# qiutang98/chord

Measured on AMD Instinct MI355X. Metric: Gtri/s into 4K 64-bit visbuffer, higher is better.
Workload: dtype f32+u64; 1 GPU; street_4k_hzb; scene_triangles_lod0=2799616, objects=352, hzb=True, cull=flat, parallelism=single

## Files before the change

chord_amd/csrc/chordvis_abi.cpp:

```cpp

#include "device_layer.h"
#include "material_tables.h"

#include <algorithm>
#include <cmath>
#include <cstddef>
#include <cstdio>
#include <cstring>

using namespace chord;

namespace chord {

int fail(ChordCtx* ctx, int code, const char* what, hipError_t e)
{
    if (ctx) {
        char buf[512];
        if (e != hipSuccess) std::snprintf(buf, sizeof(buf), "%s: %s (%d)", what, hipGetErrorString(e), (int)e);
        else std::snprintf(buf, sizeof(buf), "%s", what);
        ctx->lastError = buf;
    }
    return code;
}

}

namespace {

template <typename T>
int dalloc(ChordCtx* c, T** p, size_t count)
{
    if (*p) { (void)hipFree(*p); *p = nullptr; }
    if (count == 0) count = 1;
    CHORD_HIP(c, hipMalloc((void**)p, count * sizeof(T)));
    return CHORDVIS_OK;
}

template <typename T>
void dfree(T*& p) { if (p) { (void)hipFree((void*)p); p = nullptr; } }

uint32_t tex_block_bytes(uint32_t format)
{
    if (format == CHORD_TEXFMT_BC1_RGB || format == CHORD_TEXFMT_BC4) return 8u;
    if (format == CHORD_TEXFMT_BC3 || format == CHORD_TEXFMT_BC5) return 16u;
    return 0u;
}
#define CHORD_TEXFMT_NAMES "0 (RGBA8), 1 (BC1_RGB), 2 (BC3), 3 (BC4), 4 (BC5)"

struct TexDecodeJob {
    struct Copy { const uint8_t* host; uint64_t offset, bytes; };
    std::vector<chord::DTexLevelRec> recs;
    std::vector<Copy> copies;
    uint64_t stagingBytes = 0;
    uint32_t blocks = 0;

    void add(const ChordTexture& tx, uint32_t dst)
    {
        const uint32_t bb = tex_block_bytes(tx.format);
        const uint64_t offset = (stagingBytes + 15ull) & ~15ull;
        uint64_t bytes = 0;
        for (uint32_t l = 0; l < tx.mipCount; l++) {
            const uint32_t w = std::max(1u, tx.width >> l), h = std::max(1u, tx.height >> l), bw = (w + 3u) / 4u, bh = (h + 3u) / 4u;
            recs.push_back(chord::DTexLevelRec{blocks, (uint32_t)((offset + bytes) / 8u), dst, w, h, bw, tx.format, 0u});
            blocks += bw * bh; bytes += (uint64_t)bw * bh * bb; dst += w * h;
        }
        copies.push_back(Copy{tx.rgba8, offset, bytes});
        stagingBytes = offset + bytes;
    }

    int run(ChordCtx* c, const char* who, uint32_t* texels, uint8_t* alpha, bool alphaOnly)
    {
        if (recs.empty()) return CHORDVIS_OK;
        if (stagingBytes / 8u > 0xFFFFFFFFull) return fail(c, CHORDVIS_E_CAPACITY, "texture decode: more than 32 GiB of compressed texture levels in one upload");
        const uint32_t count = (uint32_t)recs.size();
        recs.push_back(chord::DTexLevelRec{blocks, 0u, 0u, 0u, 0u, 1u, 0u, 0u});
        uint8_t* dStaging = nullptr;
        chord::DTexLevelRec* dRecs = nullptr;
        hipError_t e = hipMalloc((void**)&dStaging, stagingBytes);
        if (e == hipSuccess) e = hipMalloc((void**)&dRecs, recs.size() * sizeof(recs[0]));
        if (e == hipSuccess) e = hipMemcpy(dRecs, recs.data(), recs.size() * sizeof(recs[0]), hipMemcpyHostToDevice);
        for (size_t i = 0; i < copies.size() && e == hipSuccess; i++)
            e = hipMemcpy(dStaging + copies[i].offset, copies[i].host, copies[i].bytes, hipMemcpyHostToDevice);
        if (e == hipSuccess) {
            chord::launch_texture_decode(c, dRecs, count, blocks, dStaging, texels, alpha, alphaOnly);
            e = hipGetLastError();
            const hipError_t es = hipStreamSynchronize(c->stream);
            if (e == hipSuccess) e = es;
        }
        if (dStaging) (void)hipFree(dStaging);
        if (dRecs) (void)hipFree(dRecs);
        return e == hipSuccess ? CHORDVIS_OK : fail(c, CHORDVIS_E_HIP, who, e);
    }
};

void record(ChordCtx* c, int tag) { chord::stamp(c, tag); }

void begin_frame_stamps(ChordCtx* c)
{
    c->frameLaunchBase = c->launchCount;
    c->stampThisFrame = c->timers && (c->frameIndex % c->timerPeriod) == 0;
    c->frameIndex++;
    if (!c->stampThisFrame) return;
    if (c->timers == 1) { c->stampTags.clear(); c->framesStamped = 0; }
    c->framesStamped++;
    chord::stamp(c, S_FRAME_BEGIN);
}

int alloc_hzb(ChordCtx* c, HzbBuffers& h)
{
    ChordHZBDesc d;
    if (chordvis_hzb_desc(c->width, c->height, &d) != CHORDVIS_OK) return fail(c, CHORDVIS_E_INVALID, "render size unsupported for HZB");
    h.desc = d;
    h.valid = false; h.uploaded = false;
    int rc;
    if ((rc = dalloc(c, &h.minTexels, d.totalTexels))) return rc;
    if ((rc = dalloc(c, &h.maxTexels, d.totalTexels))) return rc;
    if ((rc = dalloc(c, &h.validRange, 2))) return rc;
    CHORD_HIP(c, hipMemsetAsync(h.minTexels, 0, sizeof(uint16_t) * d.totalTexels, c->stream));
    CHORD_HIP(c, hipMemsetAsync(h.maxTexels, 0, sizeof(uint16_t) * d.totalTexels, c->stream));
    return CHORDVIS_OK;
}

int configure_targets(ChordCtx* c, uint64_t* external)
{
    c->resolveFrame = false;
    const uint32_t N = c->shard.ranks;
    c->tilesX = (c->width + CHORD_TILE - 1) >> CHORD_TILE_SHIFT; c->tilesY = (c->height + CHORD_TILE - 1) >> CHORD_TILE_SHIFT;
    c->shard.tilesX = c->tilesX;
    c->slotCapacity = N > 1 ? chordvis_tile_slot_capacity(c->width, c->height, N) : 0u;
    c->visWords = N > 1 ? (uint64_t)N * c->slotCapacity * (CHORD_TILE * CHORD_TILE) : (uint64_t)c->width * c->height;
    int rc;
    if (external) {
        dfree(c->dVisOwned);
        c->dVis = external; c->visExternal = true;
    } else {
        if ((rc = dalloc(c, &c->dVisOwned, c->visWords))) return rc;
        c->dVis = c->dVisOwned; c->visExternal = false;
    }
    if (N > 1) { if ((rc = dalloc(c, &c->dVisResolved, (uint64_t)c->width * c->height))) return rc; }
    else dfree(c->dVisResolved);
    for (int i = 0; i < 3; i++) if ((rc = alloc_hzb(c, c->hzb[i]))) return rc;
    c->historySlot = 0;
    c->pendingTailSlot = 0;
    {
        c->binCap = CHORD_BIN_CAP;
        if ((rc = dalloc(c, &c->dTileBins, (size_t)2 * c->tilesX * c->tilesY * c->binCap))) return rc;
        c->binPoolChunks = c->limitPoolChunks;
        if ((rc = dalloc(c, &c->dBinPool, (size_t)2 * c->binPoolChunks * CHORD_BIN_CHUNK))) return rc;
        const size_t tabWords = (size_t)2 * c->tilesX * c->tilesY * c->binMaxChunks;
        if ((rc = dalloc(c, &c->dBinChunkTab, tabWords))) return rc;
        CHORD_HIP(c, hipMemset(c->dBinChunkTab, 0, tabWords * sizeof(unsigned long long)));
        const size_t tilesN = (size_t)c->tilesX * c->tilesY;
        c->tileItemCap = (uint32_t)(tilesN * (CHORD_TILE_MAX_SLICES + 1u));
        if ((rc = dalloc(c, &c->dTileOrder, ((size_t)1 + c->tileItemCap) * 2))) return rc;
        if ((rc = dalloc(c, &c->dTileOrderKeep, ((size_t)1 + c->tileItemCap) * 4))) return rc;
        if ((rc = dalloc(c, &c->dTileOrderKeep1, ((size_t)1 + c->tileItemCap) * 4))) return rc;
        c->orderAge = c->orderAge1 = 0xFFFFFFFFu;
        if ((rc = dalloc(c, &c->dTileSlabs, tilesN * CHORD_TILE * CHORD_TILE))) return rc;
        CHORD_HIP(c, hipMemset(c->dTileSlabs, 0, tilesN * CHORD_TILE * CHORD_TILE * sizeof(unsigned long long)));
    }
    if ((rc = dalloc(c, &c->dTileRange, (size_t)2 * CHORD_MAX_TILES))) return rc;
    if (!c->hBinHint) {
        void* h = nullptr; void* dh = nullptr;
        CHORD_HIP(c, hipHostMalloc(&h, 64, hipHostMallocMapped));
        std::memset(h, 0, 64);
        CHORD_HIP(c, hipHostGetDevicePointer(&dh, h, 0));
        c->hBinHint = static_cast<volatile uint32_t*>(h); c->dBinHint = static_cast<uint32_t*>(dh);
    }
    if (c->dHotTiles) CHORD_HIP(c, hipMemsetAsync(c->dHotTiles, 0, sizeof(uint32_t) * 2 * (1 + CHORD_HOT_TILES), c->stream));
    c->hBinHint[0] = 0u; c->hBinHint[1] = 0u;
    c->hBinHint[2] = 0xFFFFFFFFu; c->hBinHint[3] = 0xFFFFFFFFu;
    for (int k = 4; k < 8; k++) c->hBinHint[k] = 0u;
    {
        const uint32_t vw = (c->width + 1) / 2, vh = (c->height + 1) / 2;
        if ((rc = dalloc(c, &c->dRangePartials, (size_t)((vw + 63) / 64) * ((vh + 3) / 4) * 2))) return rc;
    }
    if (N > 1) {
        const size_t tilesN = (size_t)c->tilesX * c->tilesY;
        CHORD_HIP(c, hipMemsetAsync(c->dVis, 0, c->visWords * 8, c->stream));
        if ((rc = dalloc(c, &c->dShardTables, 64 + (tilesN + 1) / 2))) return rc;
        if ((rc = dalloc(c, &c->dTileLoads, tilesN))) return rc;
        CHORD_HIP(c, hipMemsetAsync(c->dTileLoads, 0, tilesN * 4, c->stream));
        if (c->tileOwners.size() != tilesN || !c->tileOwnersExplicit) {
            c->tileOwners.assign(tilesN, 0);
            c->tileOwnersExplicit = false;
            if (tile_layout(c->tilesX, c->tilesY, N, nullptr, 0u, c->tileOwners.data()) != CHORDVIS_OK) return fail(c, CHORDVIS_E_INVALID, "tile layout");
        }
        const size_t slots = (size_t)N * c->slotCapacity;
        if ((rc = dalloc(c, &c->dHzbExchange, slots * CHORD_HZB_SLOT_HALVES))) return rc;
        CHORD_HIP(c, hipMemsetAsync(c->dHzbExchange, 0, slots * CHORD_HZB_SLOT_HALVES * 2, c->stream));
        if ((rc = dalloc(c, &c->dHzbFinalExchange, slots * CHORD_HZB_FINAL_SLOT_HALVES))) return rc;
        CHORD_HIP(c, hipMemsetAsync(c->dHzbFinalExchange, 0, slots * CHORD_HZB_FINAL_SLOT_HALVES * 2, c->stream));
        if ((rc = install_tile_owners(c))) return rc;
        if ((rc = prepare_cull_exchange(c))) return rc;
    } else {
        dfree(c->dHzbExchange); dfree(c->dHzbFinalExchange); dfree(c->dShardTables); dfree(c->dTileLoads); dfree(c->dTileOwner); dfree(c->dCullExchange);
        c->shard.ownedRows = nullptr; c->shard.tileSlot = nullptr;
        c->hzbExchangeHalves = c->hzbExchangeChunkHalves = 0; c->hzbFinalExchangeChunkBytes = 0;
    }
    dfree(c->dVisAlt); dfree(c->dVisResolvedAlt);
    return CHORDVIS_OK;
}

HzbBuffers from_handle(const ChordHZB* h)
{
    HzbBuffers b;
    b.desc = h->desc; b.minTexels = h->minTexels; b.maxTexels = h->maxTexels; b.validRange = h->validRange;
    b.valid = h->minTexels != nullptr;
    return b;
}

CmdList from_handle(const ChordCountAndCmd& h)
{
    CmdList l; l.count = h.count; l.cmds = h.cmds; l.capacity = h.capacity; return l;
}

int ready(ChordCtx* c, const char* fn)
{
    if (!c) return CHORDVIS_E_INVALID;
    if (!c->sceneLoaded || !c->viewSet || !c->dVis) {
        char buf[160];
        std::snprintf(buf, sizeof(buf), "%s: upload_scene, allocate_gbuffer and set_view must come first", fn);
        return fail(c, CHORDVIS_E_INVALID, buf);
    }
    return CHORDVIS_OK;
}

int flush_view(ChordCtx* c)
{
    if (c->viewDirty) {
        CHORD_HIP(c, hipMemcpyAsync(c->dView, &c->hView, sizeof(DView), hipMemcpyHostToDevice, c->stream));
        c->viewDirty = false;
    }
    if (c->zeroFrameStateInCull) {
        CHORD_HIP(c, hipMemsetAsync(c->dFrameState, 0, c->frameStateZeroBytes, c->stream));
        c->zeroFrameStateInCull = false;
    }
    return CHORDVIS_OK;
}

int flush_pending_tail(ChordCtx* c)
{
    if (c->pendingTailSlot) {
        launch_hzb_tail(c, c->hzb[c->pendingTailSlot], true, true);
        c->pendingTailSlot = 0;
        CHORD_HIP(c, hipGetLastError());
    }
    return CHORDVIS_OK;
}

int begin_frame_clear(ChordCtx* c)
{
    c->frameStateZeroBytes = offsetof(FrameState, tileCount) + sizeof(uint32_t) * CHORD_TILECOUNT_STRIDE * ((size_t)2 * c->tilesX * c->tilesY);
    c->zeroFrameStateInCull = true;
    c->rasterCalls = 0;
    c->pendingClear = true;
    c->inFrame = true;
    return CHORDVIS_OK;
}

int do_raster(ChordCtx* c, const CmdList& in)
{
    const hipError_t e = launch_raster(c, in, c->pendingClear);
    c->pendingClear = false;
    if (e != hipSuccess) return fail(c, CHORDVIS_E_HIP, "launch_raster", e);
    CHORD_HIP(c, hipGetLastError());
    c->resolveFrame = true; c->resolveStale = false;
    return CHORDVIS_OK;
}

}

namespace chord {
void stamp(ChordCtx* c, int tag)
{
    if (!c->timers || !c->stampThisFrame) return;
    const size_t i = c->stampTags.size();
    if (i >= c->evPool.size()) {
        hipEvent_t e;
        if (hipEventCreate(&e) != hipSuccess) return;
        c->evPool.push_back(e);
    }
    (void)hipEventRecord(c->evPool[i], c->stream);
    c->stampTags.push_back(tag);
}
}

namespace chord {
int install_tile_owners(ChordCtx* c)
{
    const uint32_t N = c->shard.ranks, tiles = c->tilesX * c->tilesY;
    if (N <= 1 || !c->dShardTables || c->tileOwners.size() != tiles) return fail(c, CHORDVIS_E_INVALID, "tile owners: no sharded G-buffer");
    std::vector<uint32_t> used(N, 0);
    for (uint32_t t = 0; t < tiles; t++) {
        const uint32_t o = c->tileOwners[t];
        if (o >= N || ++used[o] > c->slotCapacity) return fail(c, CHORDVIS_E_INVALID, "tile owners: an owner out of range, or a rank with more tiles than chordvis_tile_slot_capacity");
    }
    const uint32_t S = *std::max_element(used.begin(), used.end());
    std::vector<unsigned long long> tab(64 + (tiles + 1) / 2, 0ull);
    uint32_t* slot = reinterpret_cast<uint32_t*>(tab.data() + 64);
    std::fill(used.begin(), used.end(), 0u);
    for (uint32_t t = 0; t < tiles; t++) {
        const uint32_t o = c->tileOwners[t];
        slot[t] = o * S + used[o]++;
        if (o == c->shard.rank) tab[t / c->tilesX] |= 1ull << (t % c->tilesX);
    }
    c->shard.slotsPerRank = S;
    c->hzbExchangeChunkHalves = (uint64_t)S * CHORD_HZB_SLOT_HALVES;
    c->hzbExchangeHalves = c->hzbExchangeChunkHalves * N;
    c->hzbFinalExchangeChunkBytes = (uint64_t)S * CHORD_HZB_FINAL_SLOT_HALVES * 2;
    CHORD_HIP(c, hipMemcpyAsync(c->dShardTables, tab.data(), tab.size() * sizeof(unsigned long long), hipMemcpyHostToDevice, c->stream));
    CHORD_HIP(c, hipStreamSynchronize(c->stream));
    c->shard.ownedRows = c->dShardTables;
    c->shard.tileSlot = reinterpret_cast<const uint32_t*>(c->dShardTables + 64);
    if (c->dTileOwner) { (void)hipFree(c->dTileOwner); c->dTileOwner = nullptr; }
    CHORD_HIP(c, hipMalloc((void**)&c->dTileOwner, tiles));
    CHORD_HIP(c, hipMemcpy(c->dTileOwner, c->tileOwners.data(), tiles, hipMemcpyHostToDevice));
    c->mineValid = false; c->listMine[1] = c->listMine[2] = false;
    c->orderAge = c->orderAge1 = 0xFFFFFFFFu;
    return CHORDVIS_OK;
}

int ensure_cull_exchange(ChordCtx* c)
{
    if (!c->sceneLoaded || c->shard.ranks <= 1 || c->shard.ranks > 8u) return fail(c, CHORDVIS_E_INVALID, "cull exchange: a scene on a context sharded over 2..8 ranks");
    const uint32_t N = c->shard.ranks, chunkBlocks = (c->cullBlocks + N - 1u) / N;
    if (c->dCullExchange && c->cullChunkBlocks == chunkBlocks && c->cullExchangeRanks == N) return CHORDVIS_OK;
    CHORD_HIP(c, hipStreamSynchronize(c->stream));
    if (c->dCullExchange) { (void)hipFree(c->dCullExchange); c->dCullExchange = nullptr; }
    const size_t words = (size_t)N * chunkBlocks * 257u;
    CHORD_HIP(c, hipMalloc((void**)&c->dCullExchange, words * 4u));
    CHORD_HIP(c, hipMemsetAsync(c->dCullExchange, 0, words * 4u, c->stream));
    c->cullChunkBlocks = chunkBlocks; c->cullExchangeRanks = N;
    return CHORDVIS_OK;
}

int prepare_cull_exchange(ChordCtx* c)
{
    if (!c->sceneLoaded || c->shard.ranks <= 1 || c->shard.ranks > 8u) return CHORDVIS_OK;
    return ensure_cull_exchange(c);
}

int alloc_scene_work_buffers(ChordCtx* c)
{
    int rc;
    const uint64_t instTriangles = c->instTriangles;
    if ((rc = dalloc(c, &c->dObjectsOwned, (size_t)c->objectCount))) return rc;
    if ((rc = dalloc(c, &c->dObjFrame, (size_t)c->objectCount))) return rc;
    if ((rc = dalloc(c, &c->dGroupMask, (size_t)c->groupInstances + 16))) return rc;
    if ((rc = dalloc(c, &c->dBlockCounts, (size_t)c->cullBlocks * 3))) return rc;
    c->fullListStale = false;
    for (int i = 0; i < 3; i++) {
        if ((rc = dalloc(c, &c->lists[i].cmds, (size_t)c->cmdCapacity))) return rc;
        c->lists[i].count = c->dCounts + i;
        c->lists[i].capacity = c->cmdCapacity;
    }
    const uint64_t need = (2 * instTriangles + (256u << 10) + CHORD_LIST_SHARDS - 1) & ~(uint64_t)(CHORD_LIST_SHARDS - 1);
    c->triCapC = (uint32_t)std::min<uint64_t>(c->limitRecords, need);
    c->triCap = (uint32_t)std::min<uint64_t>(std::max<uint64_t>(c->limitRecords / 4, 1u << 20), need) & ~(CHORD_LIST_SHARDS - 1u);
    c->clipTriCap = 1u << 20;
    if ((rc = dalloc(c, &c->dTris, (size_t)c->triCap))) return rc;
    if ((rc = dalloc(c, &c->dTrisC, (size_t)c->triCapC))) return rc;
    c->blockCap = (uint32_t)std::min<uint64_t>((uint64_t)c->triCapC * 2u / CHORD_LIST_SHARDS, CHORD_REC_INDEX_MASK / CHORD_LIST_SHARDS);
    if ((rc = dalloc(c, &c->dBlockPool, (size_t)c->blockCap * CHORD_LIST_SHARDS * 2u))) return rc;
    if ((rc = dalloc(c, &c->dClipTris, (size_t)c->clipTriCap))) return rc;
    c->largeCap = 8u << 20;
    if ((rc = dalloc(c, &c->dLargeList, (size_t)c->largeCap))) return rc;
    return CHORDVIS_OK;
}
}

extern "C" {


int chordvis_create(int deviceOrdinal, void* hipStream, ChordCtx** outCtx)
{
    if (!outCtx) return CHORDVIS_E_INVALID;
    *outCtx = nullptr;
    int n = 0;
    if (hipGetDeviceCount(&n) != hipSuccess || n <= 0 || deviceOrdinal < 0 || deviceOrdinal >= n) return CHORDVIS_E_NO_DEVICE;
    ChordCtx* c = new ChordCtx();
    c->device = deviceOrdinal;
    if (hipSetDevice(deviceOrdinal) != hipSuccess) { delete c; return CHORDVIS_E_NO_DEVICE; }
    hipDeviceProp_t prop;
    if (hipGetDeviceProperties(&prop, deviceOrdinal) == hipSuccess) c->numCUs = prop.multiProcessorCount > 0 ? prop.multiProcessorCount : 256;
    if (hipStream) { c->stream = (hipStream_t)hipStream; c->ownStream = false; }
    else {
        if (hipStreamCreateWithFlags(&c->stream, hipStreamNonBlocking) != hipSuccess) { delete c; return CHORDVIS_E_HIP; }
        c->ownStream = true;
    }
    bool ok = hipMalloc((void**)&c->dTileClocks, sizeof(unsigned long long) * 18 * CHORD_MAX_TILES) == hipSuccess &&
              hipMalloc((void**)&c->dHotTiles, sizeof(uint32_t) * 2 * (1 + CHORD_HOT_TILES)) == hipSuccess &&
              hipMemset(c->dHotTiles, 0, sizeof(uint32_t) * 2 * (1 + CHORD_HOT_TILES)) == hipSuccess &&
              hipMalloc((void**)&c->dView, sizeof(DView)) == hipSuccess &&
              hipMalloc((void**)&c->dFrameState, sizeof(FrameState)) == hipSuccess;
    if (!ok) { chordvis_destroy(c); return CHORDVIS_E_HIP; }
    c->dCounters = &c->dFrameState->counters;
    c->dCounts = c->dFrameState->listCounts;
    (void)hipMemsetAsync(c->dFrameState, 0, sizeof(FrameState), c->stream);
    *outCtx = c;
    return CHORDVIS_OK;
}

int chordvis_destroy(ChordCtx* c)
{
    if (!c) return CHORDVIS_E_INVALID;
    (void)hipSetDevice(c->device);
    (void)hipStreamSynchronize(c->stream);
    (void)chordvis_comm_destroy(c);
    if (c->depthCtx) { chordvis_destroy(c->depthCtx); c->depthCtx = nullptr; }
    for (float*& d : c->dDepthImages) dfree(d);
    if (c->sharedScene) {
        c->dPrims = nullptr; c->dGroups = nullptr; c->dMeshlets = nullptr; c->dGroupIndices = nullptr; c->dMeshletData = nullptr;
        c->dPositions = nullptr; c->dObjStatic = nullptr; c->dGroupRefs = nullptr; c->dMaterials = nullptr; c->dTexAlpha = nullptr;
        c->dTexcoords = nullptr; c->dBvhNodes = nullptr; c->dMeshletLod = nullptr; c->dNormals = nullptr; c->dTangents = nullptr;
        c->dMatRecords = nullptr; c->dMatTexels = nullptr;
    }
    dfree(c->dPrims); dfree(c->dGroups); dfree(c->dMeshlets); dfree(c->dGroupIndices); dfree(c->dMeshletData);
    dfree(c->dPositions); dfree(c->dObjStatic); dfree(c->dMaterials); dfree(c->dTexAlpha); dfree(c->dTexcoords); dfree(c->dBvhNodes); dfree(c->dGroupRefs); dfree(c->dObjectsOwned); dfree(c->dMeshletLod);
    dfree(c->dNormals); dfree(c->dTangents); dfree(c->dMatRecords); dfree(c->dMatTexels);
    dfree(c->dView); dfree(c->dObjFrame); dfree(c->dGroupMask); dfree(c->dBlockCounts);
    for (int i = 0; i < 3; i++) dfree(c->lists[i].cmds);
    dfree(c->dRankCmds); dfree(c->dLeftCmds); dfree(c->dMineCmds);
    dfree(c->dCullLookback);
    dfree(c->dFrameState); c->dCounts = nullptr; c->dCounters = nullptr; dfree(c->dTileClocks); dfree(c->dHotTiles); dfree(c->dTileOrder); dfree(c->dTileOrderKeep); dfree(c->dTileOrderKeep1); c->orderAge = c->orderAge1 = 0xFFFFFFFFu; dfree(c->dTileSlabs); dfree(c->dTileMarker); dfree(c->dShadingTiles);
    dfree(c->dVisOwned); dfree(c->dVisResolved);
    for (int i = 0; i < 3; i++) { dfree(c->hzb[i].minTexels); dfree(c->hzb[i].maxTexels); dfree(c->hzb[i].validRange); }
    if (c->hBinHint) { (void)hipHostFree(const_cast<uint32_t*>(c->hBinHint)); c->hBinHint = nullptr; c->dBinHint = nullptr; }
    dfree(c->dRangePartials); dfree(c->dTileRange); dfree(c->dHzbExchange); dfree(c->dHzbFinalExchange); dfree(c->dShardTables); dfree(c->dTileLoads); dfree(c->dTileOwner); dfree(c->dCullExchange); dfree(c->dVisAlt); dfree(c->dVisResolvedAlt); dfree(c->dTris); dfree(c->dTrisC); dfree(c->dBlockPool); dfree(c->dTileBins); dfree(c->dBinPool); dfree(c->dBinChunkTab);
    dfree(c->dClipTris); dfree(c->dLargeList);
    for (hipEvent_t e : c->evPool) (void)hipEventDestroy(e);
    if (c->ownStream && c->stream) (void)hipStreamDestroy(c->stream);
    delete c;
    return CHORDVIS_OK;
}

const char* chordvis_last_error(ChordCtx* c) { return c ? c->lastError.c_str() : "null context"; }

int chordvis_sync(ChordCtx* c)
{
    if (!c) return CHORDVIS_E_INVALID;
    { const int rc = flush_pending_tail(c); if (rc) return rc; }
    CHORD_HIP(c, hipStreamSynchronize(c->stream));
    return CHORDVIS_OK;
}


int chordvis_upload_scene(ChordCtx* c, const ChordSceneDesc* s)
{
    if (c) c->orderAge = c->orderAge1 = 0xFFFFFFFFu;

    if (!c || !s || !s->objects || !s->primitives || !s->materials || !s->assets || s->objectCount == 0)
        return fail(c, CHORDVIS_E_INVALID, "upload_scene: null or empty scene");
    CHORD_HIP(c, hipSetDevice(c->device));

    std::vector<uint32_t> mB(s->assetCount + 1, 0), gB(s->assetCount + 1, 0), iB(s->assetCount + 1, 0), dB(s->assetCount + 1, 0), vB(s->assetCount + 1, 0);
    for (uint32_t a = 0; a < s->assetCount; a++) {
        const ChordAssetDesc& as = s->assets[a];
        if (!as.meshlets || !as.meshletGroups || !as.meshletGroupIndices || !as.meshletData || !as.positions)
            return fail(c, CHORDVIS_E_INVALID, "upload_scene: asset with null stream");
        mB[a + 1] = mB[a] + as.meshletCount; gB[a + 1] = gB[a] + as.meshletGroupCount;
        iB[a + 1] = iB[a] + as.meshletGroupIndexCount; dB[a + 1] = dB[a] + as.meshletDataCount; vB[a + 1] = vB[a] + as.vertexCount;
    }
    {
        uint64_t verts = 0;
        for (uint32_t a = 0; a < s->assetCount; a++) verts += s->assets[a].vertexCount;
        if (verts > 0x55555555ull) return fail(c, CHORDVIS_E_INVALID, "upload_scene: more than 0x55555555 vertices in one scene");
    }
    const uint32_t nM = mB.back(), nG = gB.back(), nI = iB.back(), nD = dB.back(), nV = vB.back();
    std::vector<uint32_t> nB(s->assetCount + 1, 0);
    for (uint32_t a = 0; a < s->assetCount; a++) nB[a + 1] = nB[a] + (s->assets[a].bvhNodes ? s->assets[a].bvhNodeCount : 0u);
    std::vector<DBVHNode> bvh(nB.back());
    bool bvhComplete = nB.back() > 0;

    std::vector<DMeshlet> meshlets(nM);
// ... 1447 lines not shown
```

chord_amd/csrc/kernels_raster.hip:

```cpp

#include "device_layer.h"
#include "device_math.h"
#include "texel_wrap.h"

#include <algorithm>
#include <cstdlib>
#include <cstring>
#include <type_traits>

namespace chord {

#define GUARD_BAND 1024.0f
#define LDS_VERTS 256
#define TILE CHORD_TILE
#define TILE_SHIFT CHORD_TILE_SHIFT
#define TPITCH (TILE + 1)
#define SMALL_AREA 256
#define TC_STRIDE CHORD_TILECOUNT_STRIDE
#define TC_BLOCKS 1u
#define TC_TICKET 2u
#define TC_MASKED 3u

struct RasterParams {
    const uint32_t* count; const ChordDrawCmd* cmds;
    uint32_t cmdCap;
    uint32_t* leftCount; ChordDrawCmd* leftCmds;
    const DObjFrame* objFrame; const DObjStatic* objStatic;
    const DMeshlet* meshlets; const uint32_t* meshletData; const float* positions;
    const DMaterial* materials; const uint8_t* texAlpha; const float* texcoords;
    unsigned long long* vis;
    float* depthOut;
    float W, H; int32_t Wi, Hi;
    ShardInfo shard;
    TriRec* tris; uint32_t triCap;
    TriRecC* trisC; uint32_t triCapC;
    uint32_t* tileCount; uint32_t* tileBins; uint32_t binCap; uint32_t tilesX, tilesY;
    uint32_t* binPool; uint32_t binPoolChunks; uint32_t* binPoolCount;
    unsigned long long* binChunkTab; uint32_t binStamp; uint32_t binMaxChunks;
    unsigned long long* blockPool; uint32_t blockCap;
    uint32_t blockForce;
    ClipTri* clipTris; uint32_t clipTriCap; uint32_t pass;
    uint32_t* largeList; uint32_t largeCap;
    uint32_t binInSetup;
    DeviceCounters* counters;
    uint2* tileOrder;
    unsigned long long* tileSlabs;
    uint32_t hzbFused;
    ChordHZBDesc hzbDesc;
    uint16_t* hzbMinA;
    uint16_t* hzbMinB; uint16_t* hzbMaxB;
    uint16_t* hzbExA;
    uint16_t* hzbExB;
    uint32_t* tileRange;
    unsigned long long* tileClocks;
    unsigned long long* tilePhase;
    uint32_t depthOnly, depthClamp;
    float biasConst, biasSlope;
    uint32_t clearTiles;
    uint32_t* binHint;
    uint32_t* countHint;
    uint32_t slotHot;
    uint32_t* hotTiles;
    uint32_t tileSlots;
    uint32_t tileSplitMin, tileSliceLen;
    uint2* tileOrderNext;
    uint32_t orderAll;
    uint32_t orderKept;
    uint32_t* heavyHint;
    uint32_t* tileTouched;
    uint32_t debug;
    uint32_t wideMax;
};
#define ABL(p, flag) (RASTER_ABLATION && ((p).debug & (flag)) != 0u)
#define DBG_NO_PIXELS   1u
#define DBG_NO_BIN      2u
#define DBG_TILE_CLOCKS 16u
#define DBG_NO_OUT      128u
#define DBG_NO_HZB      256u
#define DBG_SETUP_CLOCKS 512u
#define DBG_NO_VIS_STORE 1024u
#define DBG_NO_SPLIT    2048u
#define DBG_NO_TINY     32u
#define DBG_TILE_EXIT   64u
#define DBG_NO_ENTRY    8192u
#define DBG_NO_BATCH    16384u
#define DBG_NO_UNITS    4096u
#define DBG_SKIP_LIGHT  1048576u
#define DBG_SKIP_HEAVY  2097152u

template <typename T>
__device__ __forceinline__ T scalar_load(const T* ptr)
{
    return *reinterpret_cast<const __attribute__((address_space(4))) T*>(reinterpret_cast<uintptr_t>(ptr));
}
__device__ __forceinline__ const RasterParams* kernel_args()
{
    unsigned long long kp = (unsigned long long)__builtin_amdgcn_kernarg_segment_ptr();
    asm volatile("" : "+s"(kp));
    return reinterpret_cast<const RasterParams*>(kp);
}

__device__ __forceinline__ uint32_t mbcnt64(unsigned long long m) { return __builtin_amdgcn_mbcnt_hi((uint32_t)(m >> 32), __builtin_amdgcn_mbcnt_lo((uint32_t)m, 0u)); }
__device__ __forceinline__ int32_t bcast(int32_t v, int src) { return __builtin_amdgcn_readlane(v, src); }
__device__ __forceinline__ uint32_t bcast(uint32_t v, int src) { return (uint32_t)__builtin_amdgcn_readlane((int)v, src); }
__device__ __forceinline__ float bcast(float v, int src) { return __int_as_float(__builtin_amdgcn_readlane(__float_as_int(v), src)); }

__device__ __forceinline__ bool owns_tile(const ShardInfo& s, int32_t tx, int32_t ty)
{
    if (s.ranks <= 1) return true;
    return shard_owns_tile(s, (uint32_t)tx, (uint32_t)ty);
}
__device__ __forceinline__ bool owns_rect(const ShardInfo& s, int32_t px0, int32_t py0, int32_t px1, int32_t py1)
{
    if (s.ranks <= 1) return true;
    return shard_owns_any_tile(s, (uint32_t)px0 >> TILE_SHIFT, (uint32_t)py0 >> TILE_SHIFT, (uint32_t)px1 >> TILE_SHIFT, (uint32_t)py1 >> TILE_SHIFT);
}

__device__ __forceinline__ bool in_fast_volume_xy(const f4& h)
{
    return h.w > 0.0f && (GUARD_BAND * h.w + h.x) >= 0.0f && (GUARD_BAND * h.w - h.x) >= 0.0f &&
           (GUARD_BAND * h.w + h.y) >= 0.0f && (GUARD_BAND * h.w - h.y) >= 0.0f;
}

__device__ __forceinline__ bool in_fast_volume(const f4& h)
{
    return h.w > 0.0f && (h.w - h.z) >= 0.0f && h.z >= 0.0f &&
           (GUARD_BAND * h.w + h.x) >= 0.0f && (GUARD_BAND * h.w - h.x) >= 0.0f &&
           (GUARD_BAND * h.w + h.y) >= 0.0f && (GUARD_BAND * h.w - h.y) >= 0.0f;
}

struct TriSetup {
    int32_t X[3], Y[3];
    float d0, e1, e2, invA;
    int32_t px0, py0, px1, py1;
    int64_t area;
    int32_t s;
    uint32_t payload;
};

__device__ __forceinline__ bool narrow_extent(const TriSetup& ts)
{
    const int32_t extX = max(ts.X[0], max(ts.X[1], ts.X[2])) - min(ts.X[0], min(ts.X[1], ts.X[2]));
    const int32_t extY = max(ts.Y[0], max(ts.Y[1], ts.Y[2])) - min(ts.Y[0], min(ts.Y[1], ts.Y[2]));
    return extX <= (1 << 14) && extY <= (1 << 14);
}

__device__ __forceinline__ bool fits_compact(const TriSetup& ts)
{
    return narrow_extent(ts);
}

__device__ __forceinline__ void write_record_c(TriRecC* dst, const TriSetup& ts, const float d[3])
{
    TriRecC r;
    r.X0 = ts.X[0]; r.Y0 = ts.Y[0];
    r.dX1 = (int16_t)(ts.X[1] - ts.X[0]); r.dY1 = (int16_t)(ts.Y[1] - ts.Y[0]);
    r.dX2 = (int16_t)(ts.X[2] - ts.X[0]); r.dY2 = (int16_t)(ts.Y[2] - ts.Y[0]);
    r.d[0] = d[0]; r.d[1] = d[1]; r.d[2] = d[2];
    r.payload = ts.payload;
    *dst = r;
}

__device__ __forceinline__ bool tri_setup(TriSetup& ts, bool twoSided, int32_t Wi, int32_t Hi)
{
    const int32_t dx1 = ts.X[1] - ts.X[0], dy1 = ts.Y[1] - ts.Y[0], dx2 = ts.X[2] - ts.X[0], dy2 = ts.Y[2] - ts.Y[0];
    int64_t area2;
    const bool small = (uint32_t)(dx1 + 32767) < 65535u && (uint32_t)(dy1 + 32767) < 65535u &&
                       (uint32_t)(dx2 + 32767) < 65535u && (uint32_t)(dy2 + 32767) < 65535u;
    const bool allSmall = __ballot(!small) == 0ull;
    if (allSmall) area2 = (int64_t)(__mul24(dx1, dy2) - __mul24(dx2, dy1));
    else area2 = (int64_t)dx1 * (int64_t)dy2 - (int64_t)dx2 * (int64_t)dy1;
    if (area2 == 0) return false;
    if (!twoSided && area2 > 0) return false;
    ts.s = area2 < 0 ? -1 : 1;
    ts.area = area2 < 0 ? -area2 : area2;
    const int32_t minX = min(ts.X[0], min(ts.X[1], ts.X[2])), maxX = max(ts.X[0], max(ts.X[1], ts.X[2]));
    const int32_t minY = min(ts.Y[0], min(ts.Y[1], ts.Y[2])), maxY = max(ts.Y[0], max(ts.Y[1], ts.Y[2]));
    ts.px0 = max(0, (minX + 127) >> 8);
    ts.py0 = max(0, (minY + 127) >> 8);
    ts.px1 = min(Wi - 1, (maxX - 128) >> 8);
    ts.py1 = min(Hi - 1, (maxY - 128) >> 8);
    if (ts.px1 < ts.px0 || ts.py1 < ts.py0) return false;
    if (allSmall) ts.invA = 1.0f / (float)(int32_t)ts.area;
    else ts.invA = 1.0f / (float)(double)ts.area;
    return true;
}

__device__ __forceinline__ float depth_bias(const TriSetup& ts, const float d[3], float biasConst, float biasSlope)
{
    const int64_t s = ts.s;
    const float invA = ts.invA;
    const int64_t a1 = -s * (int64_t)(ts.Y[0] - ts.Y[2]), b1 = s * (int64_t)(ts.X[0] - ts.X[2]);
    const int64_t a2 = -s * (int64_t)(ts.Y[1] - ts.Y[0]), b2 = s * (int64_t)(ts.X[1] - ts.X[0]);
    const float e1 = d[1] - d[0], e2 = d[2] - d[0];
    const float dzdx = ((float)(double)(a1 * 256) * invA) * e1 + ((float)(double)(a2 * 256) * invA) * e2;
    const float dzdy = ((float)(double)(b1 * 256) * invA) * e1 + ((float)(double)(b2 * 256) * invA) * e2;
    const float m = fmaxf(fabsf(dzdx), fabsf(dzdy));
    const float mz = fmaxf(fabsf(d[0]), fmaxf(fabsf(d[1]), fabsf(d[2])));
    const int32_t e = (int32_t)((__float_as_uint(mz) >> 23) & 0xFFu) - 23;
    const float r = (e > 0 && e < 255) ? __uint_as_float((uint32_t)e << 23) : 0.0f;
    return biasSlope * m + biasConst * r;
}

__device__ __forceinline__ void tri_setup_from_compact(TriSetup& ts, const TriRecC& r, int32_t Wi, int32_t Hi)
{
    ts.X[0] = r.X0; ts.Y[0] = r.Y0;
    ts.X[1] = r.X0 + r.dX1; ts.Y[1] = r.Y0 + r.dY1;
    ts.X[2] = r.X0 + r.dX2; ts.Y[2] = r.Y0 + r.dY2;
    ts.payload = r.payload;
    const int32_t area2 = (int32_t)r.dX1 * (int32_t)r.dY2 - (int32_t)r.dX2 * (int32_t)r.dY1;
    ts.s = area2 < 0 ? -1 : 1;
    ts.invA = 1.0f / (float)(area2 < 0 ? -area2 : area2);
    ts.d0 = r.d[0]; ts.e1 = r.d[1] - r.d[0]; ts.e2 = r.d[2] - r.d[0];
    const int32_t minX = min(ts.X[0], min(ts.X[1], ts.X[2])), maxX = max(ts.X[0], max(ts.X[1], ts.X[2]));
    const int32_t minY = min(ts.Y[0], min(ts.Y[1], ts.Y[2])), maxY = max(ts.Y[0], max(ts.Y[1], ts.Y[2]));
    ts.px0 = max(0, (minX + 127) >> 8);
    ts.py0 = max(0, (minY + 127) >> 8);
    ts.px1 = min(Wi - 1, (maxX - 128) >> 8);
    ts.py1 = min(Hi - 1, (maxY - 128) >> 8);
    ts.area = 0;
}

__device__ __forceinline__ void tri_setup_from_record(TriSetup& ts, const TriRec& r, int32_t Wi, int32_t Hi)
{
#pragma unroll
    for (int i = 0; i < 3; i++) { ts.X[i] = r.X[i]; ts.Y[i] = r.Y[i]; }
    ts.payload = r.payload;
    ts.s = (r.twoSided & 2u) ? -1 : 1;
    ts.invA = __uint_as_float(r.pad);
    ts.d0 = r.d[0]; ts.e1 = r.d[1] - r.d[0]; ts.e2 = r.d[2] - r.d[0];
    const int32_t minX = min(ts.X[0], min(ts.X[1], ts.X[2])), maxX = max(ts.X[0], max(ts.X[1], ts.X[2]));
    const int32_t minY = min(ts.Y[0], min(ts.Y[1], ts.Y[2])), maxY = max(ts.Y[0], max(ts.Y[1], ts.Y[2]));
    ts.px0 = max(0, (minX + 127) >> 8);
    ts.py0 = max(0, (minY + 127) >> 8);
    ts.px1 = min(Wi - 1, (maxX - 128) >> 8);
    ts.py1 = min(Hi - 1, (maxY - 128) >> 8);
    ts.area = 0;
}



struct RecordEmitParams {
    DeviceCounters* counters; ClipTri* clipTris; uint32_t clipTriCap; uint32_t pass;
    TriRec* tris; uint32_t triCap; TriRecC* trisC; uint32_t triCapC; uint32_t* largeList; uint32_t largeCap;
    uint32_t* tileCount; uint32_t* tileBins; uint32_t binCap; uint32_t tilesX;
    uint32_t* binPool; uint32_t binPoolChunks; uint32_t* binPoolCount;
    unsigned long long* binChunkTab; uint32_t binStamp; uint32_t binMaxChunks;
    uint32_t* tileTouched;
    uint32_t binInSetup;
    ShardInfo shard;
};
__device__ __forceinline__ RecordEmitParams load_record_emit_params()
{
    const RasterParams* q = kernel_args();
    RecordEmitParams e;
    e.counters = scalar_load(&q->counters); e.clipTris = scalar_load(&q->clipTris); e.clipTriCap = scalar_load(&q->clipTriCap); e.pass = scalar_load(&q->pass);
    e.tris = scalar_load(&q->tris); e.triCap = scalar_load(&q->triCap); e.trisC = scalar_load(&q->trisC); e.triCapC = scalar_load(&q->triCapC);
    e.largeList = scalar_load(&q->largeList); e.largeCap = scalar_load(&q->largeCap);
    e.tileCount = scalar_load(&q->tileCount); e.tileBins = scalar_load(&q->tileBins); e.binCap = scalar_load(&q->binCap); e.tilesX = scalar_load(&q->tilesX);
    e.binPool = scalar_load(&q->binPool); e.binPoolChunks = scalar_load(&q->binPoolChunks); e.binPoolCount = scalar_load(&q->binPoolCount);
    e.binChunkTab = scalar_load(&q->binChunkTab); e.binStamp = scalar_load(&q->binStamp); e.binMaxChunks = scalar_load(&q->binMaxChunks);
    e.tileTouched = scalar_load(&q->tileTouched); e.binInSetup = scalar_load(&q->binInSetup);
    e.shard.ranks = scalar_load(&q->shard.ranks); e.shard.rank = scalar_load(&q->shard.rank); e.shard.slotsPerRank = 0u; e.shard.tilesX = 0u;
    e.shard.ownedRows = scalar_load(&q->shard.ownedRows); e.shard.tileSlot = nullptr;
    return e;
}

struct BinElect { int leader; uint32_t rank, group; };

__device__ __forceinline__ BinElect wave_bin_elect(bool has, uint32_t tile, uint32_t lane)
{
    BinElect e; e.leader = 0; e.rank = 0; e.group = 0;
    unsigned long long todo = __ballot(has);
    const unsigned long long lt = (1ull << lane) - 1ull;
    while (todo) {
        const int l = __ffsll((long long)todo) - 1;
        const uint32_t k = bcast(tile, l);
        const unsigned long long same = __ballot(has && tile == k);
        if (has && tile == k) { e.leader = l; e.rank = (uint32_t)__popcll(same & lt); e.group = (uint32_t)__popcll(same); }
        todo &= ~same;
    }
    return e;
}

__device__ __forceinline__ uint32_t bin_capacity(const RasterParams& p) { return p.binCap + p.binMaxChunks * CHORD_BIN_CHUNK; }

template <class P>
__device__ __forceinline__ void bin_alloc(const P& p, uint32_t tile, uint32_t slot)
{
    if (slot == 0u && p.tileTouched) atomicOr(&p.tileTouched[tile >> 5], 1u << (tile & 31u));
    if (slot < p.binCap) return;
    const uint32_t o = slot - p.binCap, j = o >> CHORD_BIN_CHUNK_SHIFT;
    if (j >= p.binMaxChunks || (o & (CHORD_BIN_CHUNK - 1u)) != 0u) return;
    uint32_t id = atomicAdd(p.binPoolCount, 1u);
    if (id >= p.binPoolChunks) { id = CHORD_BIN_CHUNK_INVALID; atomicOr(&p.counters->overflow, 1u); }
    __hip_atomic_store(p.binChunkTab + (__umul24(tile, p.binMaxChunks) + j), ((unsigned long long)p.binStamp << 32) | id,
                       __ATOMIC_RELAXED, __HIP_MEMORY_SCOPE_AGENT);
}

template <class P>
__device__ __forceinline__ void bin_put(const P& p, uint32_t tile, uint32_t slot, uint32_t gi)
{
    if (slot < p.binCap) { p.tileBins[__umul24(tile, p.binCap) + slot] = gi; return; }
    const uint32_t o = slot - p.binCap, j = o >> CHORD_BIN_CHUNK_SHIFT;
    if (j >= p.binMaxChunks) { atomicOr(&p.counters->overflow, 1u); return; }
    const unsigned long long* ent = p.binChunkTab + (__umul24(tile, p.binMaxChunks) + j);
    const unsigned long long stamp = (unsigned long long)p.binStamp << 32;
    unsigned long long e = 0;
    uint32_t spins = 0;
    for (;;) {
        e = __hip_atomic_load(ent, __ATOMIC_RELAXED, __HIP_MEMORY_SCOPE_AGENT);
        if ((e & 0xFFFFFFFF00000000ull) == stamp) break;
        if (++spins > (1u << 20)) { atomicOr(&p.counters->overflow, 4u); return; }
        __builtin_amdgcn_s_sleep(4);
    }
    const uint32_t id = (uint32_t)e;
    if (id != CHORD_BIN_CHUNK_INVALID) p.binPool[((size_t)id << CHORD_BIN_CHUNK_SHIFT) + (o & (CHORD_BIN_CHUNK - 1u))] = gi;
}

template <class P>
__device__ __forceinline__ void bin_store(const P& p, uint32_t tile, uint32_t slot, uint32_t gi)
{
    bin_alloc(p, tile, slot);
    bin_put(p, tile, slot, gi);
}

struct BinTicket {
    uint32_t tileA[4], tileB[4], slotA[4], slotB[4];
    uint32_t has;
    uint32_t eA[4], eB[4];
};

template <class P>
__device__ __forceinline__ void wave_bin_issue(const P& p, bool emitA, const TriSetup& tsA, bool emitB, const TriSetup& tsB,
                                               uint32_t lane, BinTicket& k, const bool masked = false)
{
    auto tile_of = [&](const TriSetup& ts, int r, bool emit, uint32_t& tile) -> bool {
        const int32_t tx0 = ts.px0 >> TILE_SHIFT, tx1 = ts.px1 >> TILE_SHIFT, ty0 = ts.py0 >> TILE_SHIFT, ty1 = ts.py1 >> TILE_SHIFT;
        const int32_t tx = (r & 1) ? tx1 : tx0, ty = (r & 2) ? ty1 : ty0;
        bool has = emit && !((r & 1) && tx1 == tx0) && !((r & 2) && ty1 == ty0);
        if (has) has = owns_tile(p.shard, tx, ty);
        tile = has ? __umul24((uint32_t)ty, p.tilesX) + (uint32_t)tx : 0u;
        return has;
    };
    k.has = 0u;
#pragma unroll
    for (int r = 0; r < 4; r++) {
        k.slotA[r] = 0u; k.slotB[r] = 0u;
        if (tile_of(tsA, r, emitA, k.tileA[r])) k.has |= 1u << r;
        if (tile_of(tsB, r, emitB, k.tileB[r])) k.has |= 16u << r;
    }
#pragma unroll
    for (int r = 0; r < 4; r++) {
        const BinElect a = wave_bin_elect((k.has & (1u << r)) != 0u, k.tileA[r], lane);
        const BinElect b = wave_bin_elect((k.has & (16u << r)) != 0u, k.tileB[r], lane);
        k.eA[r] = (uint32_t)a.leader | a.rank << 8; k.eB[r] = (uint32_t)b.leader | b.rank << 8;
        if ((k.has & (1u << r)) && (int)lane == a.leader) k.slotA[r] = atomicAdd(&p.tileCount[(size_t)k.tileA[r] * TC_STRIDE], a.group);
        if ((k.has & (16u << r)) && (int)lane == b.leader) k.slotB[r] = atomicAdd(&p.tileCount[(size_t)k.tileB[r] * TC_STRIDE], b.group);
    }
    if (masked) {
#pragma unroll
        for (int r = 0; r < 4; r++) {
            if ((k.has & (1u << r)) && lane == (k.eA[r] & 0xFFu)) p.tileCount[(size_t)k.tileA[r] * TC_STRIDE + TC_MASKED] = 1u;
            if ((k.has & (16u << r)) && lane == (k.eB[r] & 0xFFu)) p.tileCount[(size_t)k.tileB[r] * TC_STRIDE + TC_MASKED] = 1u;
        }
    }
}

template <class P>
__device__ __forceinline__ void wave_bin_commit(const P& p, BinTicket& k, bool okA, uint32_t giA, bool okB, uint32_t giB)
{
#pragma unroll
    for (int r = 0; r < 4; r++) {
        k.slotA[r] = __shfl(k.slotA[r], (int)(k.eA[r] & 0xFFu), 64) + (k.eA[r] >> 8);
// ... 1245 lines not shown
                rankR[r] = atomicAdd(&sCnt[h], 1u);
            }
        }
        __syncthreads();
        const uint32_t nClip = sWave[0][0] + sWave[1][0] + sWave[2][0] + sWave[3][0];
        const uint32_t nLg = sWave[0][3] + sWave[1][3] + sWave[2][3] + sWave[3][3];
        {
            uint32_t n[4], key[4], base[4];
#pragma unroll
            for (int i = 0; i < 4; i++) { n[i] = sCnt[tid + 256u * i]; key[i] = sKey[tid + 256u * i]; }
            uint32_t cbase = 0u, ebaseC = 0u, ebaseW = 0u;
            if (tid == 0u) {
                const uint32_t nEc = sWave[0][1] + sWave[1][1] + sWave[2][1] + sWave[3][1];
                const uint32_t nEw = sWave[0][2] + sWave[1][2] + sWave[2][2] + sWave[3][2];
                if (nClip) cbase = atomicAdd(&p.counters->clipTriCount[p.pass], nClip);
                if (nEc) ebaseC = atomicAdd(&p.counters->triCountC[listShard * CHORD_SHARD_STRIDE], nEc);
                if (nEw) ebaseW = atomicAdd(&p.counters->triCount[listShard * CHORD_SHARD_STRIDE], nEw * (masked ? 1u + CHORD_MASK_EXT_SLOTS : 1u));
                if (nLg) atomicAdd(&p.counters->largeCount[p.pass][listShard * CHORD_SHARD_STRIDE], nLg);
            }
#pragma unroll
            for (int i = 0; i < 4; i++) base[i] = n[i] ? atomicAdd(&p.tileCount[(size_t)key[i] * TC_STRIDE], n[i]) : 0u;
            if (MASKED && masked) {
#pragma unroll
                for (int i = 0; i < 4; i++) if (n[i]) p.tileCount[(size_t)key[i] * TC_STRIDE + TC_MASKED] = 1u;
            }
#pragma unroll
            for (int i = 0; i < 4; i++) if (n[i]) sCnt[tid + 256u * i] = base[i];
            if (tid == 0u) {
                sBase[0] = cbase; sBase[1] = ebaseC; sBase[2] = ebaseW;
                if (nClip) {
                    const uint32_t r = sClip[0];
                    if (r < CLIP_RANGES) { sClip[1u + r] = cbase | (nClip - 1u) << 25; sClip[0] = r + 1u; } else atomicOr(&p.counters->overflow, 2u);
                }
            }
        }
        __syncthreads();
        {
            uint32_t offClip = 0u, offC = 0u, offW = 0u;
            for (uint32_t w = 0; w < wave; w++) { offClip += sWave[w][0]; offC += sWave[w][1]; offW += sWave[w][2]; }
            const uint32_t wSlots = masked ? 1u + CHORD_MASK_EXT_SLOTS : 1u;
            uint32_t slotR[4];
#pragma unroll
            for (int r = 0; r < 4; r++) slotR[r] = (has & (1u << r)) ? sCnt[hR[r]] + rankR[r] : 0u;
            if (kind == K_CLIP) {
                const uint32_t k = sBase[0] + offClip + (uint32_t)__popcll(cm & lt);
                if (k < p.clipTriCap) { ClipTri ct; ct.objectId = hdr.objectId; ct.meshletId = hdr.meshletId; ct.slot = hdr.slot; ct.tri = t; p.clipTris[k] = ct; }
                else atomicOr(&p.counters->overflow, 2u);
            }
            uint32_t gi = 0u;
            bool ok = false;
            if (cp) {
                const uint32_t li = sBase[1] + offC + (uint32_t)__popcll(ec & lt);
                if (li < p.triCapC) { gi = listShard * p.triCapC + li; write_record_c(&p.trisC[gi], ts, d); ok = true; }
                else atomicOr(&p.counters->overflow, 1u);
            } else if (kind == K_EMIT) {
                const uint32_t li = sBase[2] + wSlots * (offW + (uint32_t)__popcll(ew & lt));
                if (li + wSlots <= p.triCap) {
                    gi = listShard * p.triCap + li; write_record(&p.tris[gi], ts, d, twoSided, masked);
                    if (MASKED && masked) setup_emit_mask_ext(p, &p.tris[gi + 1u], triWord, uv, lW, CHORD_MATFLAG_MATERIAL(hdr.matFlags), ts.area);
                    gi |= (MASKED && masked) ? CHORD_REC_MASKED : CHORD_REC_WIDE; ok = true;
                } else atomicOr(&p.counters->overflow, 1u);
            }
#pragma unroll
            for (int r = 0; r < 4; r++) if (has & (1u << r)) bin_alloc(p, tileR[r], slotR[r]);
            if (ok) {
#pragma unroll
                for (int r = 0; r < 4; r++) if (has & (1u << r)) bin_put(p, tileR[r], slotR[r], gi);
            }
            if (nLg) {
                uint32_t nt = 0u;
                if (lg && ok) {
                    large_put(LL, t, ts);
                    LL.at(LG_GI, t) = gi;
                    nt = large_tiles(LL.at(LG_BX, t), LL.at(LG_BY, t));
                }
                if (lane < 32u) sIncl[t] = nt;
            }
        }
        if (nLg) {
            __syncthreads();
            if (wave == 0u) {
                const uint32_t a = sIncl[2u * lane], b = sIncl[2u * lane + 1u];
                uint32_t incl = a + b;
#pragma unroll
                for (int dd = 1; dd < 64; dd <<= 1) { const uint32_t nb = (uint32_t)__shfl_up((int)incl, dd, 64); if (lane >= (uint32_t)dd) incl += nb; }
                sIncl[2u * lane] = incl - b; sIncl[2u * lane + 1u] = incl;
            }
            __syncthreads();
            const uint32_t total = sIncl[127];
            for (uint32_t j = tid; j < total; j += 256u) {
                uint32_t k = 0u;
#pragma unroll
                for (uint32_t st = 64u; st > 0u; st >>= 1) if (sIncl[k + st - 1u] <= j) k += st;
                const uint32_t tt = j - (k ? sIncl[k - 1u] : 0u);
                TriSetup lr;
#pragma unroll
                for (int i = 0; i < 3; i++) { lr.X[i] = (int32_t)LL.at(LG_X0 + i, k); lr.Y[i] = (int32_t)LL.at(LG_Y0 + i, k); }
                lr.s = (int32_t)LL.at(LG_S, k);
                const uint32_t bx = LL.at(LG_BX, k), by = LL.at(LG_BY, k), lgi = LL.at(LG_GI, k);
                lr.px0 = (int32_t)(bx & 0xFFFFu); lr.px1 = (int32_t)(bx >> 16); lr.py0 = (int32_t)(by & 0xFFFFu); lr.py1 = (int32_t)(by >> 16);
                const int32_t tx0 = lr.px0 >> TILE_SHIFT, ty0 = lr.py0 >> TILE_SHIFT;
                const uint32_t tw = (uint32_t)((lr.px1 >> TILE_SHIFT) - tx0 + 1);
                const int32_t tx = tx0 + (int32_t)(tt % tw), ty = ty0 + (int32_t)(tt / tw);
                const int32_t rx0 = max(lr.px0, tx << TILE_SHIFT), rx1 = min(lr.px1, (tx << TILE_SHIFT) + TILE - 1);
                const int32_t ry0 = max(lr.py0, ty << TILE_SHIFT), ry1 = min(lr.py1, (ty << TILE_SHIFT) + TILE - 1);
                const int ea[3] = {1, 2, 0}, eb[3] = {2, 0, 1};
                bool hit = owns_tile(p.shard, tx, ty);
#pragma unroll
                for (int i = 0; i < 3; i++) {
                    const int64_t dxe = (int64_t)(lr.X[eb[i]] - lr.X[ea[i]]), dye = (int64_t)(lr.Y[eb[i]] - lr.Y[ea[i]]);
                    const int64_t a = -(int64_t)lr.s * dye, b = (int64_t)lr.s * dxe;
                    const int64_t bias = (a > 0 || (a == 0 && b > 0)) ? 0 : -1;
                    const int64_t cx = (int64_t)(a > 0 ? rx1 : rx0) * 256 + 128, cy = (int64_t)(b > 0 ? ry1 : ry0) * 256 + 128;
                    hit = hit && !((int64_t)lr.s * (dxe * (cy - lr.Y[ea[i]]) - dye * (cx - lr.X[ea[i]])) + bias < 0);
                }
                if (!hit) continue;
                const uint32_t tile = (uint32_t)ty * p.tilesX + (uint32_t)tx;
                bin_store(p, tile, atomicAdd(&p.tileCount[(size_t)tile * TC_STRIDE], 1u), lgi);
                if ((lgi & 0xE0000000u) == CHORD_REC_MASKED) p.tileCount[(size_t)tile * TC_STRIDE + TC_MASKED] = 1u;
            }
        }
        __syncthreads();
        hdr = hdrN;
    }
    __syncthreads();
    if (const uint32_t ranges = sClip[0]) {
        float* a = sV[3u * wave]; float* b = sV[3u * wave + 1u]; float* cc = sV[3u * wave + 2u];
        const ClipLds<CLIP_SETUP_LANES> L = {reinterpret_cast<float4*>(a), b, b + 2u * CLIP_MAXV * CLIP_SETUP_LANES,
                                             reinterpret_cast<int32_t*>(cc), reinterpret_cast<int32_t*>(cc) + CLIP_MAXV * CLIP_SETUP_LANES,
                                             cc + 2u * CLIP_MAXV * CLIP_SETUP_LANES, lane};
        for (uint32_t i = 0; i < ranges; i++) {
            const uint32_t w = sClip[1u + i], base = w & 0x1FFFFFFu, n = (w >> 25) + 1u;
            for (uint32_t k0 = 0; k0 < n; k0 += 4u * CLIP_SETUP_LANES) {
                const uint32_t k = k0 + wave * CLIP_SETUP_LANES + lane;
                if (lane < CLIP_SETUP_LANES && k < n && base + k < p.clipTriCap) clip_entry<MASKED>(p, L, p.clipTris[base + k], listShard);
            }
        }
    }
}

template <bool HOT>
__global__ __launch_bounds__(256, BLOCKS_MIN_WAVES) void raster_setup_blocks_kernel(RasterParams p)
{
    __shared__ float sVert[6][4][BLOCKS_LDS_VERTS];
    __shared__ int32_t sSnap[2][4][BLOCKS_LDS_VERTS];
    __shared__ unsigned long long sWin[4][WIN * WIN];
    __shared__ SlotCache sSlots[HOT ? 4 : 1];
    const uint32_t count = *p.count;
    if (!launch_is_dense(p, count)) return;
    raster_setup_blocks_body<HOT>(p, count, sVert, sSnap, sWin, sSlots);
}

__device__ void raster_clip_part(const RasterParams& p, uint32_t block, uint32_t blocks)
{
    __shared__ float4 sPoly[2 * CLIP_MAXV * CLIP_THREADS];
    __shared__ float sPU[2 * CLIP_MAXV * CLIP_THREADS], sPV[2 * CLIP_MAXV * CLIP_THREADS];
    __shared__ int32_t sPX[CLIP_MAXV * CLIP_THREADS], sPY[CLIP_MAXV * CLIP_THREADS];
    __shared__ float sPD[CLIP_MAXV * CLIP_THREADS];
    if (threadIdx.x >= CLIP_THREADS) return;
    const ClipLds<CLIP_THREADS> L = {sPoly, sPU, sPV, sPX, sPY, sPD, threadIdx.x};
    const uint32_t n = min(p.counters->clipTriCount[p.pass], p.clipTriCap);
    const uint32_t listShard = block % CHORD_LIST_SHARDS;
    for (uint32_t k = block * CLIP_THREADS + threadIdx.x; k < n; k += blocks * CLIP_THREADS) {
        clip_entry<true>(p, L, p.clipTris[k], listShard);
    }
}

#define CLIP_BLOCKS 64u
__device__ void raster_bin_large_part(const RasterParams& p, uint32_t block, uint32_t blocks)
{
    const uint32_t lane = threadIdx.x & 63u, wave = threadIdx.x >> 6;
    __shared__ uint32_t sStart[CHORD_LIST_SHARDS + 1];
    if (threadIdx.x < 64u) {
        const uint32_t cnt = min(p.counters->largeCount[p.pass][threadIdx.x * CHORD_SHARD_STRIDE], p.largeCap);
        uint32_t incl = cnt;
#pragma unroll
        for (int d = 1; d < 64; d <<= 1) { const uint32_t nb = (uint32_t)__shfl_up((int)incl, d, 64); if (lane >= (uint32_t)d) incl += nb; }
        sStart[threadIdx.x + 1u] = incl;
        if (threadIdx.x == 0u) sStart[0] = 0u;
    }
    __syncthreads();
    const uint32_t n = sStart[CHORD_LIST_SHARDS];
    for (uint32_t k = block * 4u + wave; k < n; k += blocks * 4u) {
        uint32_t sh = 0;
#pragma unroll
        for (uint32_t st = 32u; st > 0u; st >>= 1) if (sStart[sh + st] <= k) sh += st;
        const uint32_t gi = __builtin_amdgcn_readfirstlane(p.largeList[(size_t)sh * p.largeCap + (k - sStart[sh])]);
        const TriRec* __restrict__ r = &p.tris[gi];
        TriSetup ts;
#pragma unroll
        for (int i = 0; i < 3; i++) { ts.X[i] = r->X[i]; ts.Y[i] = r->Y[i]; }
        ts.payload = 0;
        if (!tri_setup(ts, (r->twoSided & 1u) != 0, p.Wi, p.Hi)) continue;
        const bool maskedRec = (r->twoSided & 4u) != 0u;
        const int ea[3] = {1, 2, 0}, eb[3] = {2, 0, 1};
        int64_t a[3], b[3], bias[3], dxe[3], dye[3];
#pragma unroll
        for (int i = 0; i < 3; i++) {
            dxe[i] = (int64_t)(ts.X[eb[i]] - ts.X[ea[i]]); dye[i] = (int64_t)(ts.Y[eb[i]] - ts.Y[ea[i]]);
            a[i] = -(int64_t)ts.s * dye[i]; b[i] = (int64_t)ts.s * dxe[i];
            bias[i] = (a[i] > 0 || (a[i] == 0 && b[i] > 0)) ? 0 : -1;
        }
        const int32_t tx0 = ts.px0 >> TILE_SHIFT, tx1 = ts.px1 >> TILE_SHIFT;
        const int32_t ty0 = ts.py0 >> TILE_SHIFT, ty1 = ts.py1 >> TILE_SHIFT;
        const uint32_t tw = (uint32_t)(tx1 - tx0 + 1), nt = tw * (uint32_t)(ty1 - ty0 + 1);
        for (uint32_t tb = 0; tb < nt; tb += 64u) {
            const uint32_t t = tb + lane;
            if (t >= nt) continue;
            const int32_t tx = tx0 + (int32_t)(t % tw), ty = ty0 + (int32_t)(t / tw);
            const int32_t rx0 = max(ts.px0, tx << TILE_SHIFT), rx1 = min(ts.px1, (tx << TILE_SHIFT) + TILE - 1);
            const int32_t ry0 = max(ts.py0, ty << TILE_SHIFT), ry1 = min(ts.py1, (ty << TILE_SHIFT) + TILE - 1);
            bool hit = owns_tile(p.shard, tx, ty);
#pragma unroll
            for (int i = 0; i < 3; i++) {
                const int64_t cx = (int64_t)(a[i] > 0 ? rx1 : rx0) * 256 + 128, cy = (int64_t)(b[i] > 0 ? ry1 : ry0) * 256 + 128;
                const int64_t E = (int64_t)ts.s * (dxe[i] * (cy - ts.Y[ea[i]]) - dye[i] * (cx - ts.X[ea[i]]));
                hit = hit && !(E + bias[i] < 0);
            }
            if (hit) {
                const uint32_t tile = (uint32_t)ty * p.tilesX + (uint32_t)tx;
                const uint32_t slot = atomicAdd(&p.tileCount[(size_t)tile * TC_STRIDE], 1u);
                bin_store(p, tile, slot, gi | (maskedRec ? CHORD_REC_MASKED : CHORD_REC_WIDE));
                if (maskedRec) p.tileCount[(size_t)tile * TC_STRIDE + TC_MASKED] = 1u;
            }
        }
    }
}

__global__ __launch_bounds__(256) void raster_clip_and_bin_large_kernel(RasterParams p)
{
    if (blockIdx.x < CLIP_BLOCKS) raster_clip_part(p, blockIdx.x, CLIP_BLOCKS);
    else raster_bin_large_part(p, blockIdx.x - CLIP_BLOCKS, gridDim.x - CLIP_BLOCKS);
}

#define TILE_SLICE_SHIFT CHORD_TILE_SLICE_SHIFT
#define TILE_SLICE (1u << TILE_SLICE_SHIFT)
#ifndef TILE_SPLIT_MIN
#define TILE_SPLIT_MIN 6144u
#endif
#ifndef TILE_ORDER_KEEP
#define TILE_ORDER_KEEP 1
#endif
#ifndef TILE_DIRECT
#define TILE_DIRECT 1
#endif
#ifndef TILE_DIRECT_MAX_CLUSTERS
#define TILE_DIRECT_MAX_CLUSTERS 1024u
#endif
#ifndef TILE_SLICE_MIN
#define TILE_SLICE_MIN 1024u
#endif
template <uint32_t NT>
__device__ __forceinline__ void tile_order_part(const RasterParams& p, uint2* __restrict__ order)
{
    __shared__ uint32_t hist[20], base[20], cursor[20], splitItems, splitCursor, longest, hotCount, hotList[CHORD_HOT_TILES], entriesAll, tilesBusy;
    const uint32_t tiles = p.tilesX * p.tilesY;
    if (threadIdx.x < 20u) { hist[threadIdx.x] = 0; cursor[threadIdx.x] = 0; }
    if (threadIdx.x == 0) { splitItems = 0; splitCursor = 0; longest = 0; hotCount = 0; entriesAll = 0; tilesBusy = 0; }
    __syncthreads();
    auto tile_word = [&](uint32_t t) -> uint32_t {
        if (!owns_tile(p.shard, (int32_t)(t % p.tilesX), (int32_t)(t / p.tilesX))) return 0xFFFFFFFFu;
        const uint32_t* __restrict__ line = &p.tileCount[(size_t)t * TC_STRIDE];
        const uint32_t n = line[0], nb = line[1], nm = line[3];
        return min(n, bin_capacity(p)) | (nb ? 0x80000000u : 0u) | (nm ? 0x40000000u : 0u);
    };
    constexpr uint32_t PER_THREAD = CHORD_MAX_TILES / NT;
    uint32_t mine[PER_THREAD];
#pragma unroll
    for (uint32_t k = 0; k < PER_THREAD; k++) { const uint32_t t = threadIdx.x + k * NT; mine[k] = t < tiles ? tile_word(t) : 0xFFFFFFFFu; }
    uint32_t sumMine = 0, tilesMine = 0;
    if (p.tileSlots) {
#pragma unroll
        for (uint32_t k = 0; k < PER_THREAD; k++) {
            const uint32_t w = mine[k];
            if (w != 0xFFFFFFFFu) { const uint32_t c = w & 0x3FFFFFFFu; sumMine += c; tilesMine += c ? 1u : 0u; }
        }
        wave_sum2(sumMine, tilesMine);
        if ((threadIdx.x & 63u) == 0u) { atomicAdd(&entriesAll, sumMine); atomicAdd(&tilesBusy, tilesMine); }
        __syncthreads();
    }
    uint32_t splitMin = p.tileSplitMin, sliceLen = p.tileSliceLen;
    if (p.tileSlots && tilesBusy < p.tileSlots) {
        const uint32_t share = (entriesAll / p.tileSlots + 511u) & ~511u;
        sliceLen = min(p.tileSliceLen, max(TILE_SLICE_MIN, share));
        splitMin = min(p.tileSplitMin, sliceLen + sliceLen / 2u);
    }
    auto slices_of = [&](uint32_t c) -> uint32_t { return (c > splitMin && !ABL(p, DBG_NO_SPLIT)) ? min((c + sliceLen - 1u) / sliceLen, CHORD_TILE_MAX_SLICES) : 0u; };
#pragma unroll
    for (uint32_t k = 0; k < PER_THREAD; k++) {
        const uint32_t t = threadIdx.x + k * NT, w = mine[k];
        if (w == 0xFFFFFFFFu) continue;
        const uint32_t c = w & 0x3FFFFFFFu;
        if (c >= p.slotHot && p.hotTiles) { const uint32_t h = atomicAdd(&hotCount, 1u); if (h < CHORD_HOT_TILES) hotList[h] = t | (c >= SLOT_VERY_HOT ? 0x80000000u : 0u); }
        const uint32_t sl = slices_of(c);
        if (sl) {
            atomicAdd(&splitItems, sl);
            if (c > TILE_SPLIT_MIN) atomicMax(&longest, c);
        } else atomicAdd(&hist[c ? 16u - (31u - (uint32_t)__clz(c)) : 17u], 1u);
    }
    __syncthreads();
    if (threadIdx.x == 0) {
        uint32_t acc = splitItems;
        for (int b = 0; b < 18; b++) { base[b] = acc; acc += hist[b]; }
        order[0] = make_uint2((p.clearTiles || p.orderAll) ? acc : acc - hist[17], 0u);
        if (p.binHint) *p.binHint = longest;
        if (p.heavyHint) p.heavyHint[(splitItems != 0u || *p.count > TILE_DIRECT_MAX_CLUSTERS) ? 0 : 2] = p.binStamp;
        if (p.countHint) *p.countHint = *p.count;
        if (p.hotTiles) p.hotTiles[0] = min(hotCount, (uint32_t)CHORD_HOT_TILES);
    }
    if (p.hotTiles && threadIdx.x < min(hotCount, (uint32_t)CHORD_HOT_TILES)) p.hotTiles[1u + threadIdx.x] = hotList[threadIdx.x];
    __syncthreads();
#pragma unroll
    for (uint32_t k = 0; k < PER_THREAD; k++) {
        const uint32_t t = threadIdx.x + k * NT, w = mine[k];
        if (w == 0xFFFFFFFFu) continue;
        const uint32_t c = w & 0x3FFFFFFFu, sl = slices_of(c);
        if (sl) {
            const uint32_t pos = atomicAdd(&splitCursor, sl);
            for (uint32_t j = 0; j < sl; j++) order[1u + pos + j] = make_uint2(t | (j << 12) | ((sl - 1u) << 22), w);
        } else {
            const uint32_t b = c ? 16u - (31u - (uint32_t)__clz(c)) : 17u;
            order[1u + base[b] + atomicAdd(&cursor[b], 1u)] = make_uint2(t, w);
        }
    }
}

__device__ __noinline__ void tile_order_next_part(const RasterParams* q)
{
    tile_order_part<512u>(*q, q->tileOrderNext);
}

__global__ __launch_bounds__(1024) void raster_tile_order_kernel(RasterParams p)
{
    tile_order_part<1024u>(p, p.tileOrder);
}



struct WideEdges {
    int64_t a[3], b[3], bias[3], dx[3], dy[3];
    int32_t Xa[3], Ya[3];
    int32_t s;
};

__device__ __forceinline__ void wide_edges(const TriSetup& ts, WideEdges& w)
{
    const int ea[3] = {1, 2, 0}, eb[3] = {2, 0, 1};
    w.s = ts.s;
#pragma unroll
    for (int i = 0; i < 3; i++) {
        w.dx[i] = (int64_t)(ts.X[eb[i]] - ts.X[ea[i]]);
        w.dy[i] = (int64_t)(ts.Y[eb[i]] - ts.Y[ea[i]]);
        w.Xa[i] = ts.X[ea[i]]; w.Ya[i] = ts.Y[ea[i]];
        w.a[i] = -(int64_t)ts.s * w.dy[i];
        w.b[i] = (int64_t)ts.s * w.dx[i];
        w.bias[i] = (w.a[i] > 0 || (w.a[i] == 0 && w.b[i] > 0)) ? 0 : -1;
    }
}

__device__ __forceinline__ int64_t edge_at(const WideEdges& w, int i, int32_t px, int32_t py)
{
    const int64_t cx = (int64_t)px * 256 + 128, cy = (int64_t)py * 256 + 128;
    return (int64_t)w.s * (w.dx[i] * (cy - w.Ya[i]) - w.dy[i] * (cx - w.Xa[i]));
}

__device__ __forceinline__ void lds_write(unsigned long long* tile, int32_t lx, int32_t ly, float z, uint32_t payload)
{
    const unsigned long long packed = ((unsigned long long)__float_as_uint(z) << 32) | (unsigned long long)payload;
    atomicMax(&tile[ly * TPITCH + lx], packed);
}

template <int PITCH>
__device__ __forceinline__ void tile_raster_narrow(unsigned long long* tile, const TriSetup& ts, int32_t ox, int32_t oy,
                                                   int32_t x0, int32_t y0, int32_t x1, int32_t y1, bool noPixels, const bool clampZ)
{
    const bool neg = ts.s < 0;
    const int32_t dx0 = ts.X[2] - ts.X[1], dy0 = ts.Y[2] - ts.Y[1];
    const int32_t dx1 = ts.X[0] - ts.X[2], dy1 = ts.Y[0] - ts.Y[2];
    const int32_t dx2 = ts.X[1] - ts.X[0], dy2 = ts.Y[1] - ts.Y[0];
    const int32_t a0 = neg ? dy0 : -dy0, b0 = neg ? -dx0 : dx0;
    const int32_t a1 = neg ? dy1 : -dy1, b1 = neg ? -dx1 : dx1;
    const int32_t a2 = neg ? dy2 : -dy2, b2 = neg ? -dx2 : dx2;
    const int32_t bias0 = (a0 > 0 || (a0 == 0 && b0 > 0)) ? 0 : -1;
    const int32_t bias1 = (a1 > 0 || (a1 == 0 && b1 > 0)) ? 0 : -1;
    const int32_t bias2 = (a2 > 0 || (a2 == 0 && b2 > 0)) ? 0 : -1;
    const int32_t cx0 = x0 * 256 + 128, cy0 = y0 * 256 + 128;
    int32_t r0 = __mul24(b0, cy0 - ts.Y[1]) + __mul24(a0, cx0 - ts.X[1]) + bias0;
    int32_t r1 = __mul24(b1, cy0 - ts.Y[2]) + __mul24(a1, cx0 - ts.X[2]) + bias1;
    int32_t r2 = __mul24(b2, cy0 - ts.Y[0]) + __mul24(a2, cx0 - ts.X[0]) + bias2;
    int32_t E0 = r0, E1 = r1, E2 = r2;
    const int32_t w = x1 - x0 + 1, count = __mul24(w, y1 - y0 + 1);
    const int32_t sx0 = a0 * 256, sx1 = a1 * 256, sx2 = a2 * 256;
    const int32_t sw0 = b0 * 256 - __mul24(w - 1, sx0), sw1 = b1 * 256 - __mul24(w - 1, sx1), sw2 = b2 * 256 - __mul24(w - 1, sx2);
    int32_t col = 0;
    unsigned long long* px = tile + (y0 - oy) * PITCH + (x0 - ox);
    const unsigned long long payload = (unsigned long long)ts.payload;
    for (int32_t i = 0; i < count; i++) {
        const bool inside = (E0 | E1 | E2) >= 0 && !noPixels;
        const float l1 = (float)(E1 - bias1) * ts.invA, l2 = (float)(E2 - bias2) * ts.invA;
        float z = (ts.d0 + l1 * ts.e1) + l2 * ts.e2;
        if (clampZ) z = fminf(fmaxf(z, 0.0f), 1.0f);
        atomicMax(px, inside ? (((unsigned long long)__float_as_uint(z) << 32) | payload) : 0ull);
        col++;
        const bool wrap = col == w;
        E0 += wrap ? sw0 : sx0; E1 += wrap ? sw1 : sx1; E2 += wrap ? sw2 : sx2;
        px += wrap ? PITCH - w + 1 : 1;
        col = wrap ? 0 : col;
    }
}

#ifndef TINY_AREA
#define TINY_AREA 8
#endif
#ifndef TINY_AREA_DENSE
#define TINY_AREA_DENSE 48
#endif
#ifndef TINY_DENSE_MIN
#define TINY_DENSE_MIN 1024u
#endif

struct UnitParams {
    int32_t X[3], Y[3];
    float d0, e1, e2, invA;
    uint32_t payload;
    uint32_t box;
    int32_t skind;
};
#define TB 512
static_assert(TB == 512, "tile_order_part rounds a pass's slice length to batches of 512");
#define UNIT_CAP 4096

template <typename E_t>
__device__ __forceinline__ void scan_row(unsigned long long* __restrict__ tileRow, const UnitParams& u, int32_t ox, int32_t py,
                                         int32_t lx0, int32_t lx1, bool noPixels, const bool clampZ)
{
    const E_t s = (u.skind & 1) ? (E_t)-1 : (E_t)1;
    const E_t dx0 = (E_t)(u.X[2] - u.X[1]), dy0 = (E_t)(u.Y[2] - u.Y[1]);
    const E_t dx1 = (E_t)(u.X[0] - u.X[2]), dy1 = (E_t)(u.Y[0] - u.Y[2]);
    const E_t dx2 = (E_t)(u.X[1] - u.X[0]), dy2 = (E_t)(u.Y[1] - u.Y[0]);
    const E_t a0 = -s * dy0, b0 = s * dx0, a1 = -s * dy1, b1 = s * dx1, a2 = -s * dy2, b2 = s * dx2;
    const E_t bias0 = (a0 > 0 || (a0 == 0 && b0 > 0)) ? (E_t)0 : (E_t)-1;
    const E_t bias1 = (a1 > 0 || (a1 == 0 && b1 > 0)) ? (E_t)0 : (E_t)-1;
    const E_t bias2 = (a2 > 0 || (a2 == 0 && b2 > 0)) ? (E_t)0 : (E_t)-1;
    const E_t cx = (E_t)(ox + lx0) * (E_t)256 + (E_t)128, cy = (E_t)py * (E_t)256 + (E_t)128;
    E_t E0 = s * (dx0 * (cy - (E_t)u.Y[1]) - dy0 * (cx - (E_t)u.X[1])) + bias0;
    E_t E1 = s * (dx1 * (cy - (E_t)u.Y[2]) - dy1 * (cx - (E_t)u.X[2])) + bias1;
    E_t E2 = s * (dx2 * (cy - (E_t)u.Y[0]) - dy2 * (cx - (E_t)u.X[0])) + bias2;
    const E_t st0 = a0 * (E_t)256, st1 = a1 * (E_t)256, st2 = a2 * (E_t)256;
    float klo = 0.0f, khi = (float)(lx1 - lx0);
    {
        const float e[3] = {(float)E0, (float)E1, (float)E2}, t[3] = {(float)st0, (float)st1, (float)st2};
#pragma unroll
        for (int i = 0; i < 3; i++) {
            const float q = fminf(fmaxf(-e[i] * __builtin_amdgcn_rcpf(t[i]), -4.0f), 4096.0f);
            if (t[i] > 0.0f) klo = fmaxf(klo, floorf(q) - 1.0f);
            else if (t[i] < 0.0f) khi = fminf(khi, floorf(q) + 1.0f);
            else if (e[i] < 0.0f) khi = -1.0f;
        }
    }
    const int32_t k0 = (int32_t)klo, k1 = (int32_t)khi;
    E0 += (E_t)k0 * st0; E1 += (E_t)k0 * st1; E2 += (E_t)k0 * st2;
    unsigned long long* px = tileRow + lx0 + k0;
    const unsigned long long payload = noPixels ? 0ull : (unsigned long long)u.payload;
    for (int32_t k = k0; k <= k1; k++) {
        const bool inside = std::is_floating_point<E_t>::value ? (E0 >= (E_t)0 && E1 >= (E_t)0 && E2 >= (E_t)0)
                                                              : (((int64_t)E0 | (int64_t)E1 | (int64_t)E2) >= 0);
        const float l1 = (float)(double)(E1 - bias1) * u.invA, l2 = (float)(double)(E2 - bias2) * u.invA;
        float z = (u.d0 + l1 * u.e1) + l2 * u.e2;
        if (clampZ) z = fminf(fmaxf(z, 0.0f), 1.0f);
        const unsigned long long packed = ((unsigned long long)__float_as_uint(z) << 32) | payload;
        atomicMax(px, inside && !noPixels ? packed : 0ull);
        E0 += st0; E1 += st1; E2 += st2; px++;
    }
}

__device__ __forceinline__ uint32_t block_scan_tb(uint32_t v, uint32_t* waveSums, uint32_t* total)
{
    const uint32_t lane = threadIdx.x & 63u, wave = threadIdx.x >> 6;
    uint32_t incl = v;
#pragma unroll
    for (int d = 1; d < 64; d <<= 1) {
        const uint32_t nb = __shfl_up(incl, d, 64);
        if (lane >= (uint32_t)d) incl += nb;
    }
    if (lane == 63u) waveSums[wave] = incl;
    __syncthreads();
    uint32_t base = 0, tot = 0;
#pragma unroll
    for (uint32_t w = 0; w < TB / 64u; w++) { const uint32_t sw = waveSums[w]; if (w < wave) base += sw; tot += sw; }
    *total = tot;
    return base + incl - v;
}


#ifndef SEG_SHIFT
#define SEG_SHIFT 6
#endif
#define SEG (1 << SEG_SHIFT)
#ifndef MASKED_ROWS
#define MASKED_ROWS 1
#endif
#ifndef MASKED_SEG_SHIFT
#define MASKED_SEG_SHIFT 6
#endif
#define MASKED_SEG (1 << MASKED_SEG_SHIFT)
#define ENTRY_WORDS 13
#ifndef TILE_BATCH
#define TILE_BATCH TB
#endif
#ifndef TILE_UNIT_CAP
#define TILE_UNIT_CAP UNIT_CAP
#endif
struct EntrySoA { uint32_t w[ENTRY_WORDS][TILE_BATCH]; };
#define EF_KIND_SHIFT 24

template <typename E_t>
__device__ __forceinline__ int32_t scan_span(unsigned long long* __restrict__ tileRow, E_t E0, E_t E1, E_t E2, E_t st0, E_t st1, E_t st2,
                                          E_t bias1, E_t bias2, float d0, float e1, float e2, float invA, uint32_t payloadIn,
                                          int32_t lx0, int32_t lx1, bool noPixels, const bool clampZ = false)
{
    float klo = 0.0f, khi = (float)(lx1 - lx0);
    {
        const float e[3] = {(float)E0, (float)E1, (float)E2}, t[3] = {(float)st0, (float)st1, (float)st2};
#pragma unroll
        for (int i = 0; i < 3; i++) {
            const float q = fminf(fmaxf(-e[i] * __builtin_amdgcn_rcpf(t[i]), -4.0f), 4096.0f);
            if (t[i] > 0.0f) klo = fmaxf(klo, floorf(q) - 1.0f);
            else if (t[i] < 0.0f) khi = fminf(khi, floorf(q) + 1.0f);
            else if (e[i] < 0.0f) khi = -1.0f;
        }
    }
    const int32_t k0 = (int32_t)klo, k1 = (int32_t)khi;
    E0 += (E_t)k0 * st0; E1 += (E_t)k0 * st1; E2 += (E_t)k0 * st2;
    unsigned long long* px = tileRow + lx0 + k0;
    const unsigned long long payload = noPixels ? 0ull : (unsigned long long)payloadIn;
    for (int32_t k = k0; k <= k1; k++) {
        const bool inside = std::is_floating_point<E_t>::value ? (E0 >= (E_t)0 && E1 >= (E_t)0 && E2 >= (E_t)0)
                                                              : (((int64_t)E0 | (int64_t)E1 | (int64_t)E2) >= 0);
        const float l1 = (float)(double)(E1 - bias1) * invA, l2 = (float)(double)(E2 - bias2) * invA;
        float z = (d0 + l1 * e1) + l2 * e2;
        if (clampZ) z = fminf(fmaxf(z, 0.0f), 1.0f);
        const unsigned long long packed = ((unsigned long long)__float_as_uint(z) << 32) | payload;
        atomicMax(px, inside && !noPixels ? packed : 0ull);
        E0 += st0; E1 += st1; E2 += st2; px++;
    }
    return max(k1 - k0 + 1, 0);
}

__device__ __forceinline__ int32_t scan_span_i32(unsigned long long* __restrict__ tileRow, int32_t E0, int32_t E1, int32_t E2,
                                              int32_t st0, int32_t st1, int32_t st2, int32_t bias1, int32_t bias2,
                                              float d0, float e1, float e2, float invA, uint32_t payloadIn,
                                              int32_t lx0, int32_t lx1, bool noPixels, const bool clampZ)
{
    float klo = 0.0f, khi = (float)(lx1 - lx0);
    {
        const float e[3] = {(float)E0, (float)E1, (float)E2}, t[3] = {(float)st0, (float)st1, (float)st2};
#pragma unroll
        for (int i = 0; i < 3; i++) {
            const float q = fminf(fmaxf(-e[i] * __builtin_amdgcn_rcpf(t[i]), -4.0f), 4096.0f);
            if (t[i] > 0.0f) klo = fmaxf(klo, floorf(q) - 1.0f);
            else if (t[i] < 0.0f) khi = fminf(khi, floorf(q) + 1.0f);
            else if (e[i] < 0.0f) khi = -1.0f;
        }
    }
    const int32_t k0 = (int32_t)klo, k1 = (int32_t)khi;
    E0 += __mul24(k0, st0); E1 += __mul24(k0, st1); E2 += __mul24(k0, st2);
    int32_t U1 = E1 - bias1, U2 = E2 - bias2;
    unsigned long long* px = tileRow + lx0 + k0;
    const unsigned long long payload = noPixels ? 0ull : (unsigned long long)payloadIn;
    const int32_t kFirst = k0;
    for (int32_t k = k0; k <= k1; k += 2) {
        const bool insideA = (E0 | E1 | E2) >= 0;
        const bool insideB = ((E0 + st0) | (E1 + st1) | (E2 + st2)) >= 0;
        const float l1a = (float)U1 * invA, l2a = (float)U2 * invA;
        const float l1b = (float)(U1 + st1) * invA, l2b = (float)(U2 + st2) * invA;
        float za = (d0 + l1a * e1) + l2a * e2;
        float zb = (d0 + l1b * e1) + l2b * e2;
        if (clampZ) { za = fminf(fmaxf(za, 0.0f), 1.0f); zb = fminf(fmaxf(zb, 0.0f), 1.0f); }
        atomicMax(px, insideA && !noPixels ? (((unsigned long long)__float_as_uint(za) << 32) | payload) : 0ull);
        atomicMax(px + 1, insideB && !noPixels ? (((unsigned long long)__float_as_uint(zb) << 32) | payload) : 0ull);
        E0 += 2 * st0; E1 += 2 * st1; E2 += 2 * st2; U1 += 2 * st1; U2 += 2 * st2; px += 2;
    }
    return max(k1 - kFirst + 1, 0);
}

__device__ __forceinline__ uint32_t entry_store(EntrySoA& en, uint32_t t, const TriSetup& ts, bool narrow,
                                                int32_t ox, int32_t oy, int32_t x0, int32_t y0, int32_t x1, int32_t y1,
                                                bool masked = false, uint32_t recIndex = 0u)
{
    const bool maskedNarrow = masked && narrow;
    narrow = narrow && !masked;
    uint32_t box = (uint32_t)(x0 - ox) | ((uint32_t)(y0 - oy) << 6) | ((uint32_t)(x1 - ox) << 12) | ((uint32_t)(y1 - oy) << 18);
    if (narrow) {
        const int32_t s = ts.s;
        const int32_t dx0 = ts.X[2] - ts.X[1], dy0 = ts.Y[2] - ts.Y[1];
        const int32_t dx1 = ts.X[0] - ts.X[2], dy1 = ts.Y[0] - ts.Y[2];
        const int32_t dx2 = ts.X[1] - ts.X[0], dy2 = ts.Y[1] - ts.Y[0];
        const int32_t a0 = -s * dy0, b0 = s * dx0, a1 = -s * dy1, b1 = s * dx1, a2 = -s * dy2, b2 = s * dx2;
        const int32_t bias0 = (a0 > 0 || (a0 == 0 && b0 > 0)) ? 0 : -1;
        const int32_t bias1 = (a1 > 0 || (a1 == 0 && b1 > 0)) ? 0 : -1;
        const int32_t bias2 = (a2 > 0 || (a2 == 0 && b2 > 0)) ? 0 : -1;
        const int32_t cx = ox * 256 + 128, cy = oy * 256 + 128;
        en.w[0][t] = ((uint32_t)a0 & 0xFFFFu) | ((uint32_t)b0 << 16);
        en.w[1][t] = ((uint32_t)a1 & 0xFFFFu) | ((uint32_t)b1 << 16);
        en.w[2][t] = ((uint32_t)a2 & 0xFFFFu) | ((uint32_t)b2 << 16);
        en.w[3][t] = (uint32_t)(s * (__mul24(dx0, cy - ts.Y[1]) - __mul24(dy0, cx - ts.X[1])) + bias0);
        en.w[4][t] = (uint32_t)(s * (__mul24(dx1, cy - ts.Y[2]) - __mul24(dy1, cx - ts.X[2])) + bias1);
        en.w[5][t] = (uint32_t)(s * (__mul24(dx2, cy - ts.Y[0]) - __mul24(dy2, cx - ts.X[0])) + bias2);
        box |= (bias1 ? 1u << 26 : 0u) | (bias2 ? 1u << 27 : 0u);
    } else {
        int32_t mag = 0;
#pragma unroll
        for (int i = 0; i < 3; i++) mag = max(mag, max(abs(ts.X[i]), abs(ts.Y[i])));
        en.w[0][t] = (uint32_t)ts.X[0]; en.w[1][t] = (uint32_t)ts.X[1]; en.w[2][t] = (uint32_t)ts.X[2];
        en.w[3][t] = (uint32_t)ts.Y[0]; en.w[4][t] = (uint32_t)ts.Y[1]; en.w[5][t] = (uint32_t)ts.Y[2];
        box |= (masked ? 3u : (mag < (1 << 25) ? 1u : 2u)) << EF_KIND_SHIFT;
        box |= ts.s < 0 ? 1u << 28 : 0u;
        box |= maskedNarrow ? 1u << 29 : 0u;
        if (masked) en.w[12][t] = recIndex;
    }
    en.w[6][t] = __float_as_uint(ts.d0); en.w[7][t] = __float_as_uint(ts.e1); en.w[8][t] = __float_as_uint(ts.e2);
    en.w[9][t] = __float_as_uint(ts.invA); en.w[10][t] = ts.payload; en.w[11][t] = box;
    if (masked) return ((uint32_t)(y1 - y0) / MASKED_ROWS + 1u) * ((uint32_t)((x1 - x0) >> MASKED_SEG_SHIFT) + 1u);
    return (uint32_t)(y1 - y0 + 1) * ((uint32_t)((x1 - x0) >> SEG_SHIFT) + 1u);
}

template <typename E_t>
__device__ __forceinline__ void masked_rows(const RasterParams& p, unsigned long long* __restrict__ tileRow0, const UnitParams& u, uint32_t recIndex,
                                         int32_t ox, int32_t py0, int32_t nrows, int32_t lx0, int32_t lx1, bool noPixels, const bool clampZ)
{
    const TriRecMaskExt ext = *reinterpret_cast<const TriRecMaskExt*>(&p.tris[recIndex + 1u]);
    struct { float alphaFactor, alphaCutOff; } m = {ext.alphaFactor, ext.alphaCutOff};
    const AlphaLevel tex = alpha_level(p.texAlpha, ext);
    const E_t sgn = (u.skind & 1) ? (E_t)-1 : (E_t)1;
    const E_t dx0 = (E_t)(u.X[2] - u.X[1]), dy0 = (E_t)(u.Y[2] - u.Y[1]);
    const E_t dx1 = (E_t)(u.X[0] - u.X[2]), dy1 = (E_t)(u.Y[0] - u.Y[2]);
    const E_t dx2 = (E_t)(u.X[1] - u.X[0]), dy2 = (E_t)(u.Y[1] - u.Y[0]);
    const E_t a0 = -sgn * dy0, b0 = sgn * dx0, a1 = -sgn * dy1, b1 = sgn * dx1, a2 = -sgn * dy2, b2 = sgn * dx2;
    const E_t bias0 = (a0 > 0 || (a0 == 0 && b0 > 0)) ? (E_t)0 : (E_t)-1;
    const E_t bias1 = (a1 > 0 || (a1 == 0 && b1 > 0)) ? (E_t)0 : (E_t)-1;
    const E_t bias2 = (a2 > 0 || (a2 == 0 && b2 > 0)) ? (E_t)0 : (E_t)-1;
    const E_t cx = (E_t)(ox + lx0) * (E_t)256 + (E_t)128, cy = (E_t)py0 * (E_t)256 + (E_t)128;
    E_t R0 = sgn * (dx0 * (cy - (E_t)u.Y[1]) - dy0 * (cx - (E_t)u.X[1])) + bias0;
    E_t R1 = sgn * (dx1 * (cy - (E_t)u.Y[2]) - dy1 * (cx - (E_t)u.X[2])) + bias1;
    E_t R2 = sgn * (dx2 * (cy - (E_t)u.Y[0]) - dy2 * (cx - (E_t)u.X[0])) + bias2;
    const E_t st0 = a0 * (E_t)256, st1 = a1 * (E_t)256, st2 = a2 * (E_t)256;
    const E_t sy0 = b0 * (E_t)256, sy1 = b1 * (E_t)256, sy2 = b2 * (E_t)256;
    for (int32_t r = 0; r < nrows; r++, R0 += sy0, R1 += sy1, R2 += sy2) {
    E_t E0 = R0, E1 = R1, E2 = R2;
    unsigned long long* __restrict__ tileRow = tileRow0 + r * TPITCH;
    float klo = 0.0f, khi = (float)(lx1 - lx0);
    {
        const float e[3] = {(float)E0, (float)E1, (float)E2}, t[3] = {(float)st0, (float)st1, (float)st2};
#pragma unroll
        for (int i = 0; i < 3; i++) {
            const float q = fminf(fmaxf(-e[i] * __builtin_amdgcn_rcpf(t[i]), -4.0f), 4096.0f);
            if (t[i] > 0.0f) klo = fmaxf(klo, floorf(q) - 1.0f);
            else if (t[i] < 0.0f) khi = fminf(khi, floorf(q) + 1.0f);
            else if (e[i] < 0.0f) khi = -1.0f;
        }
    }
    const int32_t k0 = (int32_t)klo, k1 = (int32_t)khi;
    E0 += (E_t)k0 * st0; E1 += (E_t)k0 * st1; E2 += (E_t)k0 * st2;
    auto pixel = [&](E_t e0, E_t e1, E_t e2) -> unsigned long long {
        const bool inside = (e0 | e1 | e2) >= 0;
        const float l1 = std::is_same<E_t, int32_t>::value ? (float)(e1 - bias1) * u.invA : (float)(double)(e1 - bias1) * u.invA;
        const float l2 = std::is_same<E_t, int32_t>::value ? (float)(e2 - bias2) * u.invA : (float)(double)(e2 - bias2) * u.invA;
        const float l0 = (1.0f - l1) - l2;
        const float den = (l0 * ext.iw[0] + l1 * ext.iw[1]) + l2 * ext.iw[2];
        float tu = (l0 * ext.uw[0] + l1 * ext.uw[1]) + l2 * ext.uw[2];
        float tv = (l0 * ext.vw[0] + l1 * ext.vw[1]) + l2 * ext.vw[2];
        if (EXP_MASKED & 8) {
            float r = __builtin_amdgcn_rcpf(den);
            r = __builtin_fmaf(__builtin_fmaf(-den, r, 1.0f), r, r);
            float q = tu * r; q = __builtin_fmaf(__builtin_fmaf(-den, q, tu), r, q); tu = __builtin_fmaf(__builtin_fmaf(-den, q, tu), r, q);
            q = tv * r; q = __builtin_fmaf(__builtin_fmaf(-den, q, tv), r, q); tv = __builtin_fmaf(__builtin_fmaf(-den, q, tv), r, q);
        } else { tu = tu / den; tv = tv / den; }
        const float alpha = sample_alpha(tex, tu, tv);
        const bool keep = inside && !(alpha * m.alphaFactor - m.alphaCutOff < 0.0f) && !noPixels;
        float z = (u.d0 + l1 * u.e1) + l2 * u.e2;
        if (clampZ) z = fminf(fmaxf(z, 0.0f), 1.0f);
        return keep ? (((unsigned long long)__float_as_uint(z) << 32) | (unsigned long long)u.payload) : 0ull;
    };
    unsigned long long* px = tileRow + lx0 + k0;
    for (int32_t k = k0; k <= k1; k++, E0 += st0, E1 += st1, E2 += st2, px++) {
        if ((E0 | E1 | E2) < 0) continue;
        atomicMax(px, pixel(E0, E1, E2));
    }
    }
}

template <bool MASKED, bool DEPTH>
__device__ __forceinline__ int32_t entry_unit(const RasterParams& p, const EntrySoA& en, unsigned long long* tile, uint32_t e, uint32_t row, uint32_t seg,
                                           int32_t ox, int32_t oy, bool noPixels)
{
    const uint32_t box = en.w[11][e];
    const int32_t bx0 = (int32_t)(box & 63u), bx1 = (int32_t)((box >> 12) & 63u);
    const int32_t ly = (int32_t)row;
    const int32_t lx0 = bx0 + (int32_t)(seg << SEG_SHIFT), lx1 = min(bx1, lx0 + SEG - 1);
    unsigned long long* tileRow = tile + ly * TPITCH;
    const float d0 = __uint_as_float(en.w[6][e]), e1 = __uint_as_float(en.w[7][e]), e2 = __uint_as_float(en.w[8][e]);
    const float invA = __uint_as_float(en.w[9][e]);
    const uint32_t payload = en.w[10][e];
    const uint32_t kind = (box >> EF_KIND_SHIFT) & 3u;
    if (kind == 0u) {
        const uint32_t p0 = en.w[0][e], p1 = en.w[1][e], p2 = en.w[2][e];
        const int32_t a0 = (int32_t)(int16_t)(p0 & 0xFFFFu), b0 = (int32_t)p0 >> 16;
        const int32_t a1 = (int32_t)(int16_t)(p1 & 0xFFFFu), b1 = (int32_t)p1 >> 16;
        const int32_t a2 = (int32_t)(int16_t)(p2 & 0xFFFFu), b2 = (int32_t)p2 >> 16;
        const int32_t E0 = (int32_t)en.w[3][e] + (__mul24(a0, lx0) + __mul24(b0, ly)) * 256;
        const int32_t E1 = (int32_t)en.w[4][e] + (__mul24(a1, lx0) + __mul24(b1, ly)) * 256;
        const int32_t E2 = (int32_t)en.w[5][e] + (__mul24(a2, lx0) + __mul24(b2, ly)) * 256;
        return scan_span_i32(tileRow, E0, E1, E2, a0 * 256, a1 * 256, a2 * 256, (box >> 26) & 1u ? -1 : 0, (box >> 27) & 1u ? -1 : 0,
                             d0, e1, e2, invA, payload, lx0, lx1, noPixels, DEPTH);
    } else {
        UnitParams u;
        u.X[0] = (int32_t)en.w[0][e]; u.X[1] = (int32_t)en.w[1][e]; u.X[2] = (int32_t)en.w[2][e];
        u.Y[0] = (int32_t)en.w[3][e]; u.Y[1] = (int32_t)en.w[4][e]; u.Y[2] = (int32_t)en.w[5][e];
        u.d0 = d0; u.e1 = e1; u.e2 = e2; u.invA = invA; u.payload = payload; u.box = 0;
        u.skind = (int32_t)((box >> 28) & 1u) | (int32_t)(kind << 1);
        if (kind == 1u)      scan_row<double>(tileRow, u, ox, oy + ly, lx0, lx1, noPixels, DEPTH);
        else if (kind == 2u) scan_row<int64_t>(tileRow, u, ox, oy + ly, lx0, lx1, noPixels, DEPTH);
        return lx1 - lx0 + 1;
    }
}

template <bool DEPTH>
__device__ __forceinline__ void entry_unit_masked(const RasterParams& p, const EntrySoA& en, unsigned long long* tile, uint32_t e, uint32_t row, uint32_t seg,
                                                  int32_t ox, int32_t oy, bool noPixels)
{
    const uint32_t box = en.w[11][e];
    const int32_t bx0 = (int32_t)(box & 63u), bx1 = (int32_t)((box >> 12) & 63u), by1 = (int32_t)((box >> 18) & 63u);
    const int32_t ly = (int32_t)row, nrows = MASKED_ROWS == 1 ? 1 : min(MASKED_ROWS, by1 - ly + 1);
    const int32_t lx0 = bx0 + (int32_t)(seg << MASKED_SEG_SHIFT), lx1 = min(bx1, lx0 + MASKED_SEG - 1);
    UnitParams u;
    u.X[0] = (int32_t)en.w[0][e]; u.X[1] = (int32_t)en.w[1][e]; u.X[2] = (int32_t)en.w[2][e];
    u.Y[0] = (int32_t)en.w[3][e]; u.Y[1] = (int32_t)en.w[4][e]; u.Y[2] = (int32_t)en.w[5][e];
    u.d0 = __uint_as_float(en.w[6][e]); u.e1 = __uint_as_float(en.w[7][e]); u.e2 = __uint_as_float(en.w[8][e]);
    u.invA = __uint_as_float(en.w[9][e]); u.payload = en.w[10][e]; u.box = 0;
    u.skind = (int32_t)((box >> 28) & 1u) | (3 << 1);
    if ((box >> 29) & 1u) masked_rows<int32_t>(p, tile + ly * TPITCH, u, en.w[12][e], ox, oy + ly, nrows, lx0, lx1, noPixels, DEPTH);
    else                  masked_rows<int64_t>(p, tile + ly * TPITCH, u, en.w[12][e], ox, oy + ly, nrows, lx0, lx1, noPixels, DEPTH);
}

struct TileOutParams {
    ChordHZBDesc hzbDesc;
    uint16_t* hzbMinA; uint16_t* hzbMinB; uint16_t* hzbMaxB; uint32_t* tileRange;
    uint16_t* hzbExA; uint16_t* hzbExB;
    unsigned long long* vis; float* depthOut; int32_t Wi; uint32_t tilesX; uint32_t debug; uint32_t clearTiles;
};
__device__ __forceinline__ TileOutParams load_tile_out_params()
{
    const RasterParams* q = kernel_args();
    TileOutParams t;
    t.hzbDesc.srcWidth = scalar_load(&q->hzbDesc.srcWidth); t.hzbDesc.srcHeight = scalar_load(&q->hzbDesc.srcHeight);
    t.hzbDesc.width = scalar_load(&q->hzbDesc.width); t.hzbDesc.height = scalar_load(&q->hzbDesc.height);
    t.hzbDesc.mipCount = scalar_load(&q->hzbDesc.mipCount);
#pragma unroll
    for (int l = 0; l < 6; l++) t.hzbDesc.mipOffset[l] = scalar_load(&q->hzbDesc.mipOffset[l]);
    t.hzbMinA = scalar_load(&q->hzbMinA); t.hzbMinB = scalar_load(&q->hzbMinB); t.hzbMaxB = scalar_load(&q->hzbMaxB);
    t.hzbExA = scalar_load(&q->hzbExA); t.hzbExB = scalar_load(&q->hzbExB);
    t.tileRange = scalar_load(&q->tileRange); t.vis = scalar_load(&q->vis); t.depthOut = scalar_load(&q->depthOut);
    t.Wi = scalar_load(&q->Wi); t.tilesX = scalar_load(&q->tilesX); t.debug = scalar_load(&q->debug); t.clearTiles = scalar_load(&q->clearTiles);
    return t;
}

template <bool INTERIOR, bool SH>
__device__ __forceinline__ void tile_out_and_hzb_body(const TileOutParams& p, const unsigned long long* tile, float* sM2, uint32_t* sRange,
                                                      uint32_t tileId, uint32_t slotId, uint32_t binLength, int32_t ox, int32_t oy, int32_t tw, int32_t th)
{
    static_assert(TILE == 64 && TB == 512, "wave w <-> pixel rows 8w..8w+7");
    const ChordHZBDesc& d = p.hzbDesc;
    const uint32_t tX = tileId % p.tilesX, tY = tileId / p.tilesX;
    uint32_t tid = threadIdx.x;
    asm volatile("" : "+v"(tid));
    const uint32_t lane = tid & 63u, wave = tid >> 6, half = lane >> 5, l = lane & 31u;
    uint16_t* exA = SH && p.hzbExA ? p.hzbExA + (size_t)slotId * CHORD_HZB_SLOT_HALVES : nullptr;
    uint16_t* exB = SH ? p.hzbExB + (size_t)slotId * CHORD_HZB_FINAL_SLOT_HALVES : nullptr;
    auto vw = [&](uint32_t lv) { return min(max(1u, d.width >> lv), (((d.srcWidth - 1u) >> 1) >> lv) + 1u); };
    auto vh = [&](uint32_t lv) { return min(max(1u, d.height >> lv), (((d.srcHeight - 1u) >> 1) >> lv) + 1u); };
    auto put = [&](uint32_t lv, uint32_t lx, uint32_t ly, float mn, float mx) {
        const uint32_t side = 32u >> lv, gx = tX * side + lx, gy = tY * side + ly;
        if (INTERIOR || (lv < d.mipCount && gx < vw(lv) && gy < vh(lv))) {
            const uint16_t hmn = f32_to_f16(mn);
            uint16_t hmx = f32_to_f16(mx);
            if (lv == 5u) hmx = (uint16_t)(hmx + 1u);
            if (SH) {
                const uint32_t o = hzb_slot_level_offset(lv) + ly * side + lx;
                if (exA) exA[o] = hmn;
                exB[o] = hmn;
                exB[CHORD_HZB_FINAL_MAX_OFFSET + o] = hmx;
            } else {
                const size_t o = d.mipOffset[lv] + (size_t)gy * max(1u, d.width >> lv) + gx;
                if (p.hzbMinA) p.hzbMinA[o] = hmn;
                p.hzbMinB[o] = hmn;
                p.hzbMaxB[o] = hmx;
            }
        }
    };
    const uint32_t visBase = SH ? slotId << (2 * TILE_SHIFT) : (uint32_t)oy * (uint32_t)p.Wi + (uint32_t)ox;
    const uint32_t visPitch = SH ? (uint32_t)TILE : (uint32_t)p.Wi;
    uint32_t rmin = 0xFFFFFFFFu, rmax = 0u;
    float m1n = 0.0f, m1x = 0.0f;
#pragma unroll
    for (uint32_t rp = 0; rp < 2u; rp++) {
        const uint32_t q = 2u * half + rp;
        const int32_t row = (int32_t)(8u * wave + 2u * q), x2 = (int32_t)(2u * l);
        const int32_t r0 = min(row, th - 1), r1 = min(row + 1, th - 1), xa = min(x2, tw - 1), xb = min(x2 + 1, tw - 1);
        const unsigned long long v00 = tile[r0 * TPITCH + xa], v01 = tile[r0 * TPITCH + xb];
        const unsigned long long v10 = tile[r1 * TPITCH + xa], v11 = tile[r1 * TPITCH + xb];
        if (!SH && p.depthOut) {
            if (INTERIOR || x2 < tw) {
                float* dst = p.depthOut + (size_t)(oy + row) * (size_t)p.Wi + ox + x2;
                const float d00 = __uint_as_float((uint32_t)(v00 >> 32)), d01 = __uint_as_float((uint32_t)(v01 >> 32));
                const float d10 = __uint_as_float((uint32_t)(v10 >> 32)), d11 = __uint_as_float((uint32_t)(v11 >> 32));
                if (INTERIOR || row < th) { if (INTERIOR || x2 + 1 < tw) *reinterpret_cast<float2*>(dst) = make_float2(d00, d01); else dst[0] = d00; }
                if (INTERIOR || row + 1 < th) { if (INTERIOR || x2 + 1 < tw) *reinterpret_cast<float2*>(dst + p.Wi) = make_float2(d10, d11); else dst[p.Wi] = d10; }
            }
        } else
        if (!ABL(p, DBG_NO_VIS_STORE) && (INTERIOR || x2 < tw)) {
            unsigned long long* dst = p.vis + visBase + (size_t)row * visPitch + x2;
            if (INTERIOR || row < th) { if (INTERIOR || x2 + 1 < tw) *reinterpret_cast<ulonglong2*>(dst) = make_ulonglong2(v00, v01); else dst[0] = v00; }
            if (INTERIOR || row + 1 < th) { if (INTERIOR || x2 + 1 < tw) *reinterpret_cast<ulonglong2*>(dst + visPitch) = make_ulonglong2(v10, v11); else dst[visPitch] = v10; }
        }
        const float dq[4] = {__uint_as_float((uint32_t)(v00 >> 32)), __uint_as_float((uint32_t)(v01 >> 32)),
                             __uint_as_float((uint32_t)(v10 >> 32)), __uint_as_float((uint32_t)(v11 >> 32))};
#pragma unroll
        for (int k = 0; k < 4; k++) {
            const uint32_t bits = __float_as_uint(dq[k]);
            const bool drawn = dq[k] > 0.0f;
            rmax = max(rmax, drawn ? bits : 0u);
            rmin = min(rmin, (drawn && dq[k] < 1.0f) ? bits : 0xFFFFFFFFu);
        }
        const float mn = fminf(fminf(dq[0], dq[1]), fminf(dq[2], dq[3])), mx = fmaxf(fmaxf(dq[0], dq[1]), fmaxf(dq[2], dq[3]));
        put(0u, l, 4u * wave + q, mn, mx);
        if (rp == 0u) { m1n = mn; m1x = mx; } else { m1n = fminf(m1n, mn); m1x = fmaxf(m1x, mx); }
    }
    m1n = fminf(m1n, __shfl_xor(m1n, 1, 64)); m1x = fmaxf(m1x, __shfl_xor(m1x, 1, 64));
    if ((l & 1u) == 0u) put(1u, l >> 1, 2u * wave + half, m1n, m1x);
    float m2n = fminf(m1n, __shfl_xor(m1n, 2, 64)), m2x = fmaxf(m1x, __shfl_xor(m1x, 2, 64));
    m2n = fminf(m2n, __shfl_xor(m2n, 32, 64)); m2x = fmaxf(m2x, __shfl_xor(m2x, 32, 64));
    if (half == 0u && (l & 3u) == 0u) {
        put(2u, l >> 2, wave, m2n, m2x);
        sM2[wave * 8u + (l >> 2)] = m2n; sM2[64u + wave * 8u + (l >> 2)] = m2x;
    }
#pragma unroll
    for (int off = 32; off > 0; off >>= 1) {
        rmin = min(rmin, (uint32_t)__shfl_down(rmin, off, 64));
        rmax = max(rmax, (uint32_t)__shfl_down(rmax, off, 64));
    }
    if (lane == 0u) { sRange[wave * 2u] = rmin; sRange[wave * 2u + 1u] = rmax; }
    __syncthreads();
    if (wave == 0u) {
        const uint32_t x = lane & 7u, y = lane >> 3;
        float n3 = sM2[lane], x3 = sM2[64u + lane];
        n3 = fminf(n3, __shfl_xor(n3, 1, 64)); x3 = fmaxf(x3, __shfl_xor(x3, 1, 64));
        n3 = fminf(n3, __shfl_xor(n3, 8, 64)); x3 = fmaxf(x3, __shfl_xor(x3, 8, 64));
        if (!(x & 1u) && !(y & 1u)) put(3u, x >> 1, y >> 1, n3, x3);
        n3 = fminf(n3, __shfl_xor(n3, 2, 64)); x3 = fmaxf(x3, __shfl_xor(x3, 2, 64));
        n3 = fminf(n3, __shfl_xor(n3, 16, 64)); x3 = fmaxf(x3, __shfl_xor(x3, 16, 64));
        if (!(x & 3u) && !(y & 3u)) put(4u, x >> 2, y >> 2, n3, x3);
        n3 = fminf(n3, __shfl_xor(n3, 4, 64)); x3 = fmaxf(x3, __shfl_xor(x3, 4, 64));
        n3 = fminf(n3, __shfl_xor(n3, 32, 64)); x3 = fmaxf(x3, __shfl_xor(x3, 32, 64));
        if (lane == 0u) {
            put(5u, 0u, 0u, n3, x3);
            uint32_t lo = 0xFFFFFFFFu, hi = 0u;
#pragma unroll
            for (uint32_t w = 0; w < TB / 64u; w++) { lo = min(lo, sRange[2u * w]); hi = max(hi, sRange[2u * w + 1u]); }
            if (SH) {
                uint32_t* tail = reinterpret_cast<uint32_t*>(exB + CHORD_HZB_FINAL_RANGE_OFFSET);
                const uint32_t before = p.clearTiles ? 0u : tail[2];
                tail[0] = lo; tail[1] = hi; tail[2] = before + binLength; tail[3] = 0u;
            } else {
                p.tileRange[2u * tileId] = lo; p.tileRange[2u * tileId + 1u] = hi;
            }
        }
    }
}

template <bool SH>
__device__ __forceinline__ void tile_out_and_hzb(const unsigned long long* tile, float* sM2, uint32_t* sRange,
                                                 uint32_t tileId, uint32_t slotId, uint32_t binLength, int32_t ox, int32_t oy, int32_t tw, int32_t th)
{
    const TileOutParams p = load_tile_out_params();
    const ChordHZBDesc& d = p.hzbDesc;
    const uint32_t tX = tileId % p.tilesX, tY = tileId / p.tilesX;
    const uint32_t vw0 = min(max(1u, d.width), ((d.srcWidth - 1u) >> 1) + 1u), vh0 = min(max(1u, d.height), ((d.srcHeight - 1u) >> 1) + 1u);
    const bool interior = tw == TILE && th == TILE && d.mipCount > 5u && (tX + 1u) * 32u <= vw0 && (tY + 1u) * 32u <= vh0;
    if (interior) tile_out_and_hzb_body<true, SH>(p, tile, sM2, sRange, tileId, slotId, binLength, ox, oy, tw, th);
    else tile_out_and_hzb_body<false, SH>(p, tile, sM2, sRange, tileId, slotId, binLength, ox, oy, tw, th);
}

__device__ __noinline__ bool merge_slices(unsigned long long* tile, unsigned long long* slab, uint32_t* ticket, uint32_t slices,
                                          uint32_t* sTicket, uint32_t* overflow)
{
    constexpr uint32_t PER = TILE * TILE / TB;
    unsigned long long got[PER];
#pragma unroll
    for (uint32_t k = 0; k < PER; k++) {
        const uint32_t i = threadIdx.x + k * TB;
        const unsigned long long v = tile[(i >> TILE_SHIFT) * TPITCH + (i & (TILE - 1))];
        got[k] = v != 0ull ? atomicMax(slab + i, v) : 0ull;
    }
    unsigned long long seen = 0ull;
#pragma unroll
    for (uint32_t k = 0; k < PER; k++) seen |= got[k];
    if (seen == 0xFFFFFFFFFFFFFFFFull) *overflow = 8u;
    __syncthreads();
    if (threadIdx.x == 0) *sTicket = atomicAdd(ticket, 1u);
    __syncthreads();
    if (*sTicket != slices - 1u) return false;
#pragma unroll
    for (uint32_t k = 0; k < PER; k++) got[k] = atomicExch(slab + threadIdx.x + k * TB, 0ull);
#pragma unroll
    for (uint32_t k = 0; k < PER; k++) {
        const uint32_t i = threadIdx.x + k * TB;
        tile[(i >> TILE_SHIFT) * TPITCH + (i & (TILE - 1))] = got[k];
    }
    __syncthreads();
    return true;
}

__device__ __forceinline__ void merge_block_word(unsigned long long* tile, unsigned long long v, uint32_t i, uint32_t hdr, uint32_t rcp)
{
    const uint32_t w = ((hdr >> 12) & 15u) + 1u;
    const uint32_t row = (i * rcp) >> 16, col = i - row * w;
    const uint32_t lx = (hdr & 63u) + col, ly = ((hdr >> 6) & 63u) + row;
    if (v != 0ull && lx < (uint32_t)TILE && ly < (uint32_t)TILE) atomicMax(&tile[ly * TPITCH + lx], v);
}

__device__ __forceinline__ void merge_blocks(unsigned long long* tile, const unsigned long long* __restrict__ pool, unsigned long long todo,
                                             uint32_t name, uint32_t hdrLo, uint32_t hdrHi, uint32_t lane)
{
#define MB_PICK(H, R, N, SRC)                                                                                             \
    _Pragma("unroll") for (int j = 0; j < 4; j++) {                                                                       \
        const bool any = todo != 0ull;                                                                                    \
        const int l = any ? __ffsll((long long)todo) - 1 : 0;                                                             \
        todo &= todo - 1ull;                                                                             \
        H[j] = bcast(hdrLo, l); R[j] = bcast(hdrHi, l);                                                                   \
        SRC[j] = reinterpret_cast<const ulonglong2*>(pool + (size_t)(bcast(name, l) & CHORD_REC_INDEX_MASK) * 2u);        \
        N[j] = any ? (((H[j] >> 12) & 15u) + 1u) * (((H[j] >> 16) & 15u) + 1u) : 0u;                                      \
    }
#define MB_LOAD(A, N, SRC)                                                                                                \
    _Pragma("unroll") for (int j = 0; j < 4; j++) A[j] = 2u * lane <= N[j] && N[j] != 0u ? SRC[j][lane] : make_ulonglong2(0ull, 0ull);
#define MB_MERGE(A, H, R, N, SRC)                                                                                         \
    _Pragma("unroll") for (int j = 0; j < 4; j++) {                                                                       \
        if (lane != 0u) merge_block_word(tile, A[j].x, 2u * lane - 1u, H[j], R[j]);                                       \
        if (2u * lane < N[j]) merge_block_word(tile, A[j].y, 2u * lane, H[j], R[j]);                                      \
    }                                                                                                                     \
    _Pragma("unroll") for (int j = 0; j < 4; j++)                                                                         \
        for (uint32_t g = lane + 64u; 2u * g <= N[j]; g += 64u) {                                                         \
            const ulonglong2 v = SRC[j][g];                                                                               \
            merge_block_word(tile, v.x, 2u * g - 1u, H[j], R[j]);                                                         \
            if (2u * g < N[j]) merge_block_word(tile, v.y, 2u * g, H[j], R[j]);                                           \
        }
    if (!todo) return;
    uint32_t hA[4], rA[4], nA[4], hB[4], rB[4], nB[4];
    const ulonglong2* srcA[4];
    const ulonglong2* srcB[4];
    ulonglong2 aA[4], aB[4];
    MB_PICK(hA, rA, nA, srcA)
    MB_LOAD(aA, nA, srcA)
    for (;;) {
        const bool moreB = todo != 0ull;
        if (moreB) { MB_PICK(hB, rB, nB, srcB) MB_LOAD(aB, nB, srcB) }
        MB_MERGE(aA, hA, rA, nA, srcA)
        if (!moreB) break;
        const bool moreA = todo != 0ull;
        if (moreA) { MB_PICK(hA, rA, nA, srcA) MB_LOAD(aA, nA, srcA) }
        MB_MERGE(aB, hB, rB, nB, srcB)
        if (!moreA) break;
    }
#undef MB_PICK
#undef MB_LOAD
#undef MB_MERGE
}

__device__ __forceinline__ uint32_t touched_tile(const uint32_t* __restrict__ mask, uint32_t k, uint32_t g, uint32_t& total, uint32_t& tail)
{
    const uint32_t lane = threadIdx.x & 63u;
    const uint2 w = reinterpret_cast<const uint2*>(mask)[lane];
    const uint32_t c = (uint32_t)(__popc(w.x) + __popc(w.y));
    uint32_t incl = c;
#pragma unroll
    for (uint32_t d = 1u; d < 64u; d <<= 1) { const uint32_t t = __shfl_up(incl, d, 64); if (lane >= d) incl += t; }
    total = bcast(incl, 63);
    auto select = [&](uint32_t j) -> uint32_t {
        uint32_t r = j - (incl - c), m = w.x, pos = 0u;
        const uint32_t nLo = (uint32_t)__popc(w.x);
        if (r >= nLo) { r -= nLo; m = w.y; pos = 32u; }
#pragma unroll
        for (uint32_t s = 16u; s != 0u; s >>= 1) {
            const uint32_t n = (uint32_t)__popc(m & ((1u << s) - 1u));
            if (r >= n) { r -= n; m >>= s; pos += s; }
        }
        const unsigned long long holder = __ballot(incl - c <= j && j < incl);
        return holder ? bcast(lane * 64u + pos, (int)__ffsll((long long)holder) - 1) : 0u;
    };
    tail = select(g - 1u) + 1u;
    return select(k);
}

#ifndef TILE_MIN_BLOCKS
#define TILE_MIN_BLOCKS 4
#endif
template <bool SH, bool MASKED, bool DEPTH>
__global__ __launch_bounds__(TB, TILE_MIN_BLOCKS) void raster_tile_kernel(RasterParams p)
{
    __shared__ __align__(16) unsigned long long tile[TILE * TPITCH];
    __shared__ EntrySoA prm;
    __shared__ uint32_t unitList[TILE_UNIT_CAP];
    __shared__ uint32_t offs[16];
    __shared__ uint32_t waveSums[2][TB / 64];
    __shared__ uint32_t chunkTab[64];
    __shared__ uint32_t sTicket;
    if (ABL(p, DBG_TILE_EXIT) && !p.clearTiles) return;
#define TILE_SKEW (scalar_load(&kernel_args()->tileOrderNext) != nullptr ? 1u : 0u)
#define wgs (gridDim.x - TILE_SKEW)
    const uint32_t tilesAll = p.tilesX * p.tilesY;
    const uint32_t wg0 = blockIdx.x - (p.tileOrderNext != nullptr ? 1u : 0u);
    if (p.tileOrderNext && blockIdx.x == 0u) {
        tile_order_next_part(kernel_args());
        return;
    }
    const bool direct = p.orderKept == 2u;
    uint2 firstItem = make_uint2(wg0, 0u);
    uint32_t active = tilesAll;
    if (!direct) { firstItem = p.tileOrder[1u + min(wg0, tilesAll - 1u)]; active = p.tileOrder[0].x; }
    else if (p.tileTouched) {
        uint32_t touched, tail;
        firstItem.x = touched_tile(p.tileTouched, wg0, gridDim.x, touched, tail);
        active = touched > gridDim.x ? gridDim.x + tilesAll - tail : touched;
        if (active == 0u && wg0 == 0u && threadIdx.x == 0u && p.heavyHint) p.heavyHint[*p.count > TILE_DIRECT_MAX_CLUSTERS ? 0 : 2] = p.binStamp;
    }
    for (uint32_t oiw = wg0; (oiw & 0x7FFFFFFFu) < active; oiw = ((oiw & 0x7FFFFFFFu) + wgs) | 0x80000000u) {
    const uint32_t oi = oiw & 0x7FFFFFFFu;
    uint32_t tix = threadIdx.x;
    asm volatile("" : "+v"(tix));
    const uint2 itemCount = (oiw >> 31) == 0u ? firstItem : (direct ? make_uint2(oi + tilesAll - active, 0u) : p.tileOrder[1u + oi]);
    const uint32_t item = itemCount.x;
    const uint32_t tileId = item & 0xFFFu, slice = (item >> 12) & 0x3FFu, slices = (item >> 22) + 1u;
    const uint32_t* bin = p.tileBins + (size_t)tileId * p.binCap;
    const bool entryThread = TILE_BATCH == TB || tix < TILE_BATCH;
    uint32_t countWord = itemCount.y, wordSpec = 0xFFFFFFFFu;
    if (p.orderKept) {
        if (entryThread) wordSpec = bin[tix];
        const unsigned long long cnt = scalar_load(reinterpret_cast<const unsigned long long*>(&p.tileCount[(size_t)tileId * TC_STRIDE]));
        countWord = min((uint32_t)cnt, bin_capacity(p)) | ((uint32_t)(cnt >> 32) ? 0x80000000u : 0u);
    }
    const uint32_t nAll = countWord & 0x3FFFFFFFu;
    if (ABL(p, DBG_SKIP_LIGHT) && nAll < 64u) continue;
    if (ABL(p, DBG_SKIP_HEAVY) && nAll >= 64u) continue;
    if (direct) {
        if (p.heavyHint && tix == 0u) {
            if (nAll > p.tileSplitMin) p.heavyHint[0] = p.binStamp;
            if (oi == 0u) p.heavyHint[*p.count > TILE_DIRECT_MAX_CLUSTERS ? 0 : 2] = p.binStamp;
        }
        if (nAll == 0u) continue;
    }
    if (p.orderAll && !p.clearTiles && nAll == 0u) continue;
    const bool hasBlocks = (countWord >> 31) != 0u;
    const int32_t tinyArea = nAll >= TINY_DENSE_MIN ? TINY_AREA_DENSE : TINY_AREA;
    const uint32_t per = slices > 1u ? ((nAll + slices - 1u) / slices + TB - 1u) & ~(TB - 1u) : nAll;
    const uint32_t lo = slices > 1u ? min(nAll, slice * per) : 0u;
    const uint32_t n = ABL(p, DBG_NO_BATCH) ? lo : (slices > 1u ? min(nAll, lo + per) : nAll);
    const bool prof = RASTER_PROFILE && (p.debug & DBG_TILE_CLOCKS) != 0;
    const unsigned long long t0 = prof ? wall_clock64() : 0ull;
    unsigned long long ph[6] = {0, 0, 0, 0, 0, 0}, tp = t0;
    uint32_t cUnits = 0, cUnitIters = 0, cTiny = 0, cTinyIters = 0;
    unsigned long long bw[6] = {0, 0, 0, 0, 0, 0};
#define PHASE(i) do { if (prof) { const unsigned long long ta = wall_clock64(); __syncthreads(); const unsigned long long tn = wall_clock64(); bw[i] += tn - ta; ph[i] += tn - tp; tp = tn; } } while (0)
    const int32_t ox = (int32_t)(tileId % p.tilesX) * TILE, oy = (int32_t)(tileId / p.tilesX) * TILE;
    const int32_t tw = min(TILE, p.Wi - ox), th = min(TILE, p.Hi - oy);
    const bool noPixels = ABL(p, DBG_NO_PIXELS);
    auto slot_of_tile = [&]() -> uint32_t { return SH ? __builtin_amdgcn_readfirstlane(scalar_load(&kernel_args()->shard.tileSlot)[tileId]) : 0u; };
    auto vis_base = [&]() -> uint32_t { return SH ? slot_of_tile() << (2 * TILE_SHIFT) : (uint32_t)oy * (uint32_t)p.Wi + (uint32_t)ox; };
    const uint32_t visPitch = SH ? (uint32_t)TILE : (uint32_t)p.Wi;

    const bool early = n <= p.binCap && !hasBlocks;
    const uint32_t k0 = lo + tix;
    const uint32_t word0 = (early && entryThread && k0 < n) ? ((p.orderKept && slices == 1u) ? wordSpec : bin[k0]) : 0xFFFFFFFFu;

    bool rmw = false;
    if (p.hzbFused && !p.clearTiles) rmw = true;
    const bool mergeSlices = slices > 1u && (p.clearTiles || rmw);
    if (!(rmw && !mergeSlices)) {
        static_assert((TILE * TPITCH) % 2 == 0, "whole 16-byte words");
        for (uint32_t i = tix; i < TILE * TPITCH / 2; i += TB) reinterpret_cast<ulonglong2*>(tile)[i] = make_ulonglong2(0ull, 0ull);
    } else
    for (uint32_t i = tix, visBase = vis_base(); i < TILE * TILE / 2; i += TB) {
        const int32_t ly = (int32_t)(i >> (TILE_SHIFT - 1)), lx = (int32_t)(i & (TILE / 2 - 1)) * 2;
        ulonglong2 v = make_ulonglong2(0ull, 0ull);
        if (ly < th && lx < tw) {
            const unsigned long long* src = scalar_load(&kernel_args()->vis) + (size_t)(visBase + (uint32_t)ly * visPitch + (uint32_t)lx);
            if (lx + 1 < tw) v = *reinterpret_cast<const ulonglong2*>(src);
            else v.x = src[0];
        }
        tile[ly * TPITCH + lx] = v.x; tile[ly * TPITCH + lx + 1] = v.y;
    }
#define FETCH_REC(gi, a, b, c)                                                                       \
    do {                                                                                             \
        if ((gi) & CHORD_REC_WIDE) {                                                                 \
            const uint4* src_ = reinterpret_cast<const uint4*>(&p.tris[(gi) & CHORD_REC_WIDE_INDEX]); \
            a = src_[0]; b = src_[1]; c = src_[2];                                                   \
        } else {                                                                                     \
            const uint4* src_ = reinterpret_cast<const uint4*>(&p.trisC[(gi)]);                      \
            a = src_[0]; b = src_[1];                                                                \
        }                                                                                            \
    } while (0)
    uint32_t idxNext = 0xFFFFFFFFu, nameNext = 0xFFFFFFFFu;
    uint4 nq0 = make_uint4(0, 0, 0, 0), nq1 = nq0, nq2 = nq0;
    auto record_name = [](uint32_t w) -> uint32_t { return (w >= CHORD_REC_BLOCK || (!MASKED && (w & 0xE0000000u) == CHORD_REC_MASKED)) ? 0xFFFFFFFFu : w; };
    if (early) {
        nameNext = record_name(word0);
        if (nameNext != 0xFFFFFFFFu) FETCH_REC(nameNext, nq0, nq1, nq2);
        if (entryThread && k0 + TILE_BATCH < n) idxNext = record_name(bin[k0 + TILE_BATCH]);
    }
    __syncthreads();
    PHASE(0);

    uint32_t chunk0 = 0, chunkEnd = 0;
    const uint32_t chunksAll = n > p.binCap ? (n - p.binCap + CHORD_BIN_CHUNK - 1u) >> CHORD_BIN_CHUNK_SHIFT : 0u;
    auto window_load = [&](uint32_t from, uint32_t to) {
        const RasterParams* q = kernel_args();
        for (uint32_t j = from + tix; j < to; j += TB) {
            const unsigned long long e = scalar_load(&q->binChunkTab)[(size_t)tileId * scalar_load(&q->binMaxChunks) + j];
            chunkTab[j & 63u] = (uint32_t)(e >> 32) == scalar_load(&q->binStamp) ? (uint32_t)e : CHORD_BIN_CHUNK_INVALID;
        }
    };
    auto window_reset = [&]() {
        __syncthreads();
        chunk0 = lo > p.binCap ? (lo - p.binCap) >> CHORD_BIN_CHUNK_SHIFT : 0u;
        chunkEnd = min(chunksAll, chunk0 + 64u);
        window_load(chunk0, chunkEnd);
        __syncthreads();
    };
    auto window_advance = [&](uint32_t base) {
        if (chunkEnd >= chunksAll || base < p.binCap + ((chunk0 + 32u) << CHORD_BIN_CHUNK_SHIFT)) return;
        __syncthreads();
        const uint32_t to = min(chunksAll, chunkEnd + 32u);
        window_load(chunkEnd, to);
        chunk0 += 32u; chunkEnd = to;
        __syncthreads();
    };
    if (n > p.binCap) window_reset();
    const uint32_t wideLimit = p.triCap * CHORD_LIST_SHARDS, compactLimit = p.triCapC * CHORD_LIST_SHARDS;
    auto binWord = [&](uint32_t k) -> uint32_t {
        if (k < p.binCap) return bin[k];
        const uint32_t o = k - p.binCap, c = o >> CHORD_BIN_CHUNK_SHIFT;
        const uint32_t id = (c - chunk0) < (chunkEnd - chunk0) ? chunkTab[c & 63u] : CHORD_BIN_CHUNK_INVALID;
        if (id == CHORD_BIN_CHUNK_INVALID) return 0xFFFFFFFFu;
        return p.binPool[(size_t)id * CHORD_BIN_CHUNK + (o & (CHORD_BIN_CHUNK - 1u))];
    };
    if (hasBlocks && !noPixels) {
        const uint32_t blockCap = scalar_load(&kernel_args()->blockCap);
        const unsigned long long* blockPool = scalar_load(&kernel_args()->blockPool);
        const uint32_t blockLimit = blockCap * CHORD_LIST_SHARDS;
        uint32_t giNext = lo + tix < n ? binWord(lo + tix) : 0xFFFFFFFFu;
        for (uint32_t base = lo; base < n; base += TB) {
            window_advance(base);
            const uint32_t gi = giNext;
            giNext = base + TB + tix < n ? binWord(base + TB + tix) : 0xFFFFFFFFu;
            const bool isBlock = gi != 0xFFFFFFFFu && gi >= CHORD_REC_BLOCK && (gi & CHORD_REC_INDEX_MASK) < blockLimit;
            uint2 hdr = make_uint2(0u, 0u);
            if (isBlock) hdr = *reinterpret_cast<const uint2*>(blockPool + (size_t)(gi & CHORD_REC_INDEX_MASK) * 2u);
            merge_blocks(tile, blockPool, __ballot(isBlock), gi, hdr.x, hdr.y, tix & 63u);
        }
        if (n > p.binCap && chunk0 != (lo > p.binCap ? (lo - p.binCap) >> CHORD_BIN_CHUNK_SHIFT : 0u)) window_reset();
    }
    auto binEntry = [&](uint32_t k) -> uint32_t {
        const uint32_t gi = record_name(binWord(k));
        if (gi == 0xFFFFFFFFu || k < p.binCap) return gi;
        const bool okIdx = (gi & CHORD_REC_WIDE) ? (gi & CHORD_REC_WIDE_INDEX) < wideLimit : gi < compactLimit;
        return okIdx ? gi : 0xFFFFFFFFu;
    };
    if (!early) {
        idxNext = entryThread && k0 < n ? binEntry(k0) : 0xFFFFFFFFu;
        nameNext = idxNext;
        if (nameNext != 0xFFFFFFFFu) FETCH_REC(nameNext, nq0, nq1, nq2);
        idxNext = entryThread && k0 + TILE_BATCH < n ? binEntry(k0 + TILE_BATCH) : 0xFFFFFFFFu;
    }
    auto batch_setup = [&](const uint4 q0, const uint4 q1, const uint4 q2, const uint32_t name) -> uint32_t {
        const bool have = name != 0xFFFFFFFFu && !ABL(p, DBG_NO_ENTRY);
        if (prof) { volatile uint32_t sink = q1.w; (void)sink; }
        PHASE(1);
        uint32_t rows = 0;
        if (have) {
            TriSetup ts;
            if (name & CHORD_REC_WIDE) {
                TriRec w;
                w.X[0] = (int32_t)q0.x; w.X[1] = (int32_t)q0.y; w.X[2] = (int32_t)q0.z; w.Y[0] = (int32_t)q0.w;
                w.Y[1] = (int32_t)q1.x; w.Y[2] = (int32_t)q1.y;
                w.d[0] = __uint_as_float(q1.z); w.d[1] = __uint_as_float(q1.w); w.d[2] = __uint_as_float(q2.x);
                w.payload = q2.y; w.twoSided = q2.z; w.pad = q2.w;
                tri_setup_from_record(ts, w, p.Wi, p.Hi);
            } else {
                TriRecC cr;
                cr.X0 = (int32_t)q0.x; cr.Y0 = (int32_t)q0.y;
                cr.dX1 = (int16_t)(q0.z & 0xFFFFu); cr.dY1 = (int16_t)(q0.z >> 16);
                cr.dX2 = (int16_t)(q0.w & 0xFFFFu); cr.dY2 = (int16_t)(q0.w >> 16);
                cr.d[0] = __uint_as_float(q1.x); cr.d[1] = __uint_as_float(q1.y); cr.d[2] = __uint_as_float(q1.z);
                cr.payload = q1.w;
                tri_setup_from_compact(ts, cr, p.Wi, p.Hi);
            }
            {
                const int32_t x0 = max(ts.px0, ox), y0 = max(ts.py0, oy);
                const int32_t x1 = min(ts.px1, ox + tw - 1), y1 = min(ts.py1, oy + th - 1);
                if (x1 >= x0 && y1 >= y0) {
                    const bool narrow = narrow_extent(ts);
                    const bool maskedRec = MASKED && (name & CHORD_REC_WIDE) && (q2.z & 4u);
                    if (narrow && !maskedRec && (x1 - x0 + 1) * (y1 - y0 + 1) <= tinyArea) {
                        if (!ABL(p, DBG_NO_TINY)) tile_raster_narrow<TPITCH>(tile, ts, ox, oy, x0, y0, x1, y1, noPixels, DEPTH);
                        if (prof) { cTiny++; cTinyIters += (uint32_t)((x1 - x0 + 1) * (y1 - y0 + 1)); }
                    } else {
                        rows = entry_store(prm, tix, ts, narrow, ox, oy, x0, y0, x1, y1, maskedRec, name & CHORD_REC_WIDE_INDEX);
                    }
                }
            }
        }
        return rows;
    };
    auto batch_units = [&](const uint32_t rows, const uint32_t batchNo) {
        PHASE(2);
        uint32_t total;
        const bool mine3 = MASKED && rows && ((prm.w[11][tix] >> EF_KIND_SHIFT) & 3u) == 3u;
        const uint32_t rowsN = mine3 ? 0u : rows, rowsM = mine3 ? rows : 0u;
        const uint32_t offAll = block_scan_tb(rowsN | (rowsM << 16), waveSums[batchNo & 1u], &total);
        const uint32_t offN = offAll & 0xFFFFu, offM = offAll >> 16, totalM = MASKED ? total >> 16 : 0u;
        total &= 0xFFFFu;
        PHASE(3);
        auto list_units = [&](uint32_t off, uint32_t n, uint32_t r0) {
            if (!n) return;
            const uint32_t box = prm.w[11][tix];
            const uint32_t nseg = ((((box >> 12) & 63u) - (box & 63u)) >> SEG_SHIFT) + 1u, y0l = (box >> 6) & 63u;
            const uint32_t lo2 = max(off, r0), hi2 = min(off + n, r0 + TILE_UNIT_CAP);
            if (lo2 < hi2) {
                uint32_t j = lo2 - off;
                uint32_t row = y0l + (nseg == 1u ? j : nseg == 2u ? j >> 1 : nseg == 4u ? j >> 2 : j / 3u);
                uint32_t seg = nseg == 1u ? 0u : nseg == 2u ? (j & 1u) : nseg == 4u ? (j & 3u) : j % 3u;
                for (uint32_t u = lo2; u < hi2; u++) {
                    unitList[u - r0] = tix | (row << 9) | (seg << 15);
                    if (++seg == nseg) { seg = 0u; row++; }
                }
            }
        };
        for (uint32_t r0 = 0; r0 < total; r0 += TILE_UNIT_CAP) {
            list_units(offN, rowsN, r0);
            __syncthreads();
            const uint32_t nr = min(total - r0, (uint32_t)TILE_UNIT_CAP);
            for (uint32_t ui = tix; ui < nr; ui += TB) {
                const uint32_t d = unitList[ui];
                if (ABL(p, DBG_NO_UNITS)) continue;
                const int32_t trips = entry_unit<MASKED, DEPTH>(p, prm, tile, d & 511u, (d >> 9) & 63u, (d >> 15) & 3u, ox, oy, noPixels);
                if (prof) { cUnits++; cUnitIters += (uint32_t)trips; }
            }
            if (r0 + TILE_UNIT_CAP < total || totalM) __syncthreads();
        }
        for (uint32_t r0 = 0; r0 < totalM; r0 += TILE_UNIT_CAP) {
            if (rowsM) {
                const uint32_t box = prm.w[11][tix];
                const uint32_t nseg = ((((box >> 12) & 63u) - (box & 63u)) >> MASKED_SEG_SHIFT) + 1u, y0l = (box >> 6) & 63u;
                const uint32_t lo2 = max(offM, r0), hi2 = min(offM + rowsM, r0 + TILE_UNIT_CAP);
                if (lo2 < hi2) {
                    const uint32_t j = lo2 - offM, g = j / nseg;
                    uint32_t row = y0l + g * MASKED_ROWS, seg = j - g * nseg;
                    for (uint32_t u = lo2; u < hi2; u++) {
                        unitList[u - r0] = tix | (row << 9) | (seg << 15);
                        if (++seg == nseg) { seg = 0u; row += MASKED_ROWS; }
                    }
                }
            }
            __syncthreads();
            const uint32_t nr = min(totalM - r0, (uint32_t)TILE_UNIT_CAP);
            for (uint32_t ui = tix; ui < nr; ui += TB) {
                const uint32_t d = unitList[ui];
                entry_unit_masked<DEPTH>(p, prm, tile, d & 511u, (d >> 9) & 63u, (d >> 15) & 7u, ox, oy, noPixels);
            }
            if (r0 + TILE_UNIT_CAP < totalM) __syncthreads();
        }
        total |= totalM;
        if (total) __syncthreads();
        PHASE(4);
    };
    uint32_t batchNo = 0;
    for (uint32_t base = lo; base < n; base += TILE_BATCH, batchNo++) {
        window_advance(base);
        const uint32_t k = base + tix;
        const uint4 q0 = nq0, q1 = nq1, q2 = nq2;
        const uint32_t name = nameNext;
        nameNext = idxNext;
        if (nameNext != 0xFFFFFFFFu) FETCH_REC(nameNext, nq0, nq1, nq2);
        idxNext = entryThread && k + 2u * TILE_BATCH < n ? binEntry(k + 2u * TILE_BATCH) : 0xFFFFFFFFu;
        batch_units(batch_setup(q0, q1, q2, name), batchNo);
    }
    __syncthreads();

    if (mergeSlices) {
        const RasterParams* q = kernel_args();
        if (!merge_slices(tile, scalar_load(&q->tileSlabs) + (size_t)tileId * (TILE * TILE), &scalar_load(&q->tileCount)[(size_t)tileId * TC_STRIDE + TC_TICKET],
                          slices, &sTicket, &scalar_load(&q->counters)->overflow)) continue;
        if (rmw) {
            for (uint32_t i = tix, visBase = vis_base(); i < TILE * TILE / 2; i += TB) {
                const int32_t ly = (int32_t)(i >> (TILE_SHIFT - 1)), lx = (int32_t)(i & (TILE / 2 - 1)) * 2;
                if (ly >= th || lx >= tw) continue;
                const unsigned long long* src = p.vis + (size_t)(visBase + (uint32_t)ly * visPitch + (uint32_t)lx);
                tile[ly * TPITCH + lx] = max(tile[ly * TPITCH + lx], src[0]);
                if (lx + 1 < tw) tile[ly * TPITCH + lx + 1] = max(tile[ly * TPITCH + lx + 1], src[1]);
            }
        }
        __syncthreads();
    }

    if (ABL(p, DBG_NO_OUT)) {
    } else if (p.hzbFused && !ABL(p, DBG_NO_HZB)) {
        tile_out_and_hzb<SH>(tile, reinterpret_cast<float*>(&prm.w[0][0]), offs, tileId, slot_of_tile(), nAll, ox, oy, tw, th);
    } else if (p.clearTiles || p.hzbFused) {
        for (uint32_t i = tix, visBase = vis_base(); i < TILE * TILE / 2; i += TB) {
            const int32_t ly = (int32_t)(i >> (TILE_SHIFT - 1)), lx = (int32_t)(i & (TILE / 2 - 1)) * 2;
            if (ly >= th || lx >= tw) continue;
            const ulonglong2 v = make_ulonglong2(tile[ly * TPITCH + lx], tile[ly * TPITCH + lx + 1]);
            unsigned long long* dst = p.vis + (size_t)(visBase + (uint32_t)ly * visPitch + (uint32_t)lx);
            if (lx + 1 < tw) *reinterpret_cast<ulonglong2*>(dst) = v;
            else dst[0] = v.x;
        }
    } else {
        for (uint32_t i = tix, visBase = vis_base(); i < TILE * TILE; i += TB) {
            const int32_t ly = (int32_t)(i >> TILE_SHIFT), lx = (int32_t)(i & (TILE - 1));
            const unsigned long long v = tile[ly * TPITCH + lx];
            if (v != 0ull && ly < th && lx < tw) atomicMax(p.vis + (size_t)(visBase + (uint32_t)ly * visPitch + (uint32_t)lx), v);
        }
    }
    PHASE(5);
    if (prof) {
        if (tix == 0) {
            p.tileClocks[tileId] = wall_clock64() - t0;
            for (int i = 0; i < 6; i++) p.tilePhase[(size_t)tileId * 8 + i] = ph[i];
            p.tilePhase[(size_t)tileId * 8 + 6] = 0ull; p.tilePhase[(size_t)tileId * 8 + 7] = 0ull;
        }
        __syncthreads();
        atomicAdd(&p.tilePhase[(size_t)tileId * 8 + 6], ((unsigned long long)cUnits << 32) | cUnitIters);
        atomicAdd(&p.tilePhase[(size_t)tileId * 8 + 7], ((unsigned long long)cTiny << 32) | cTinyIters);
        if ((tix & 63u) == 0u) for (int i = 0; i < 6; i++) atomicAdd(&p.tilePhase[(size_t)tileId * 8 + i], bw[i] << 32);
    }
    __syncthreads();
    }
}
#undef wgs
#undef TILE_SKEW


hipError_t launch_raster(ChordCtx* c, const CmdList& in, bool clearTiles)
{
#define LR_HIP(call) do { const hipError_t e_ = (call); if (e_ != hipSuccess) return e_; } while (0)
    RasterParams p;
    p.hzbFused = 0; p.hzbMinA = nullptr; p.hzbMinB = nullptr; p.hzbMaxB = nullptr; p.tileRange = c->dTileRange;
    p.hzbExA = nullptr; p.hzbExB = nullptr;
    p.hzbDesc = c->hzb[0].desc;
    if (c->fuseHzb && c->shard.ranks == 1) {
        p.hzbFused = 1;
        p.hzbMinA = (clearTiles && c->fuseHzbTemp) ? c->hzb[0].minTexels : nullptr;
        p.hzbMinB = c->hzb[c->fuseHzbSlot].minTexels; p.hzbMaxB = c->hzb[c->fuseHzbSlot].maxTexels;
    } else if (c->fuseHzb) {
        p.hzbFused = 1;
        p.hzbExA = (clearTiles && c->fuseHzbTemp) ? c->dHzbExchange : nullptr;
        p.hzbExB = c->dHzbFinalExchange;
    }
    p.count = in.count; p.cmds = in.cmds; p.cmdCap = std::max(in.capacity, 1u);
    if (c->shard.ranks > 1) {
        bool mine = false;
        if (in.cmds == c->lists[0].cmds && c->mineValid) { p.count = c->dCounts + 4; p.cmds = c->dMineCmds; mine = true; }
        else if (in.cmds == c->dMineCmds && c->mineValid) mine = true;
        else for (int k = 1; k < 3; k++) if (in.cmds == c->lists[k].cmds && c->listMine[k]) mine = true;
        if (!mine) {
            if (!c->dRankCmds) LR_HIP(hipMalloc((void**)&c->dRankCmds, sizeof(ChordDrawCmd) * (size_t)c->cmdCapacity));
            CmdList filtered;
            filtered.count = c->dCounts + 5; filtered.cmds = c->dRankCmds; filtered.capacity = in.capacity;
            LR_HIP(hipMemsetAsync(filtered.count, 0, sizeof(uint32_t), c->stream));
            launch_rank_filter(c, in, filtered);
            p.count = filtered.count; p.cmds = filtered.cmds;
        }
    }
    p.objFrame = c->dObjFrame; p.objStatic = c->dObjStatic;
    p.meshlets = c->dMeshlets; p.meshletData = c->dMeshletData; p.positions = c->dPositions;
    p.materials = c->dMaterials; p.texAlpha = c->dTexAlpha; p.texcoords = c->dTexcoords;
    p.vis = (unsigned long long*)c->dVis;
    p.depthOut = (p.hzbFused && clearTiles) ? c->depthOutTarget : nullptr;
    p.W = (float)c->width; p.H = (float)c->height; p.Wi = (int32_t)c->width; p.Hi = (int32_t)c->height;
    p.shard = c->shard;
    p.blockPool = c->dBlockPool; p.blockCap = (c->debugFlags & DBG_NO_BLOCKS) ? 0u : c->blockCap;
    p.blockForce = (c->debugFlags & DBG_FORCE_BLOCKS) ? 1u : 0u;
    p.tris = c->dTris; p.triCap = c->triCap / CHORD_LIST_SHARDS;
    p.trisC = c->dTrisC; p.triCapC = c->triCapC / CHORD_LIST_SHARDS;
    const uint32_t tiles = c->tilesX * c->tilesY;
    const uint32_t pass = c->rasterCalls & 1u;
    p.tileCount = c->dFrameState->tileCount + (size_t)pass * tiles * TC_STRIDE;
    p.tileBins = c->dTileBins + (size_t)pass * tiles * c->binCap; p.binCap = c->binCap;
    p.binPool = c->dBinPool + (size_t)pass * c->binPoolChunks * CHORD_BIN_CHUNK; p.binPoolChunks = c->binPoolChunks;
    p.binPoolCount = &c->dCounters->binPoolCount[pass];
    p.binChunkTab = c->dBinChunkTab + (size_t)pass * tiles * c->binMaxChunks; p.binMaxChunks = c->binMaxChunks;
    p.binStamp = ++c->rasterSerial;
    p.tilesX = c->tilesX; p.tilesY = c->tilesY;
    p.clipTris = c->dClipTris + (size_t)pass * (c->clipTriCap / 2); p.clipTriCap = c->clipTriCap / 2; p.pass = pass;
    p.largeList = c->dLargeList + (size_t)pass * (c->largeCap / 2); p.largeCap = c->largeCap / 2 / CHORD_LIST_SHARDS;
    static const bool binInSetup = [] { const char* e = getenv("CHORDVIS_BIN_IN_SETUP"); return !e || atoi(e) != 0; }();
    p.binInSetup = binInSetup ? 1u : 0u;
    p.counters = c->dCounters;
    p.clearTiles = clearTiles ? 1u : 0u;
    p.depthOnly = c->depthOnly ? 1u : 0u; p.depthClamp = c->depthClamp ? 1u : 0u;
    p.biasConst = c->depthBiasConst; p.biasSlope = c->depthBiasSlope;
    p.debug = c->debugFlags;
    p.tileClocks = c->dTileClocks + (size_t)pass * CHORD_MAX_TILES;
    p.tileOrder = reinterpret_cast<uint2*>(c->dTileOrder); p.tileSlabs = c->dTileSlabs;
    p.tilePhase = c->dTileClocks + (size_t)2 * CHORD_MAX_TILES + (size_t)pass * CHORD_MAX_TILES * 8;

    if (!c->inFrame || c->rasterCalls >= 2) {
        LR_HIP(hipMemsetAsync(p.tileCount, 0, sizeof(uint32_t) * TC_STRIDE * tiles, c->stream));
        LR_HIP(hipMemsetAsync(&c->dCounters->clipTriCount[pass], 0, sizeof(uint32_t), c->stream));
        LR_HIP(hipMemsetAsync(c->dCounters->largeCount[pass], 0, sizeof(c->dCounters->largeCount[pass]), c->stream));
        LR_HIP(hipMemsetAsync(&c->dCounters->binPoolCount[pass], 0, sizeof(uint32_t), c->stream));
        if (!c->inFrame) { LR_HIP(hipMemsetAsync(c->dCounters->triCount, 0, sizeof(c->dCounters->triCount), c->stream));
                           LR_HIP(hipMemsetAsync(c->dCounters->triCountC, 0, sizeof(c->dCounters->triCountC), c->stream));
                           LR_HIP(hipMemsetAsync(c->dCounters->blockGranules, 0, sizeof(c->dCounters->blockGranules), c->stream)); }
    }

    const uint64_t rankPixels = (uint64_t)c->width * c->height / (c->shard.ranks > 1 ? c->shard.ranks : 1u);
    const bool maybeDense = p.blockCap != 0u && (p.blockForce != 0u || (uint64_t)in.capacity * 16ull >= rankPixels);
    p.leftCount = nullptr; p.leftCmds = nullptr;
    p.binHint = nullptr; p.countHint = nullptr;
    p.slotHot = (c->debugFlags & DBG_FORCE_HOT) ? 64u : SLOT_HOT;
    {
        static const int forced = [] { const char* e = getenv("CHORDVIS_TILE_SLOTS"); return e ? atoi(e) : -1; }();
        p.tileSlots = forced >= 0 ? (uint32_t)forced : c->shard.ranks > 1 ? (uint32_t)c->numCUs * (CHORD_TILE_SHIFT == 6 ? 2u : 6u) : 0u;
        static const int splitMin = [] { const char* e = getenv("CHORDVIS_TILE_SPLIT_MIN"); return e ? atoi(e) : -1; }();
        static const int sliceLen = [] { const char* e = getenv("CHORDVIS_TILE_SLICE"); return e ? atoi(e) : -1; }();
        p.tileSplitMin = splitMin > 0 ? (uint32_t)splitMin : TILE_SPLIT_MIN;
        p.tileSliceLen = sliceLen >= 512 ? ((uint32_t)sliceLen + 511u) & ~511u : TILE_SLICE;
    }
    p.hotTiles = c->dHotTiles ? c->dHotTiles + (size_t)pass * (1u + CHORD_HOT_TILES) : nullptr;
    bool blocksWorthLaunching = maybeDense;
    if (maybeDense && c->dBinHint) {
        p.countHint = c->dBinHint + 2 + pass;
        const uint32_t last = c->hBinHint[2 + pass];
        if (p.blockForce == 0u && last != 0xFFFFFFFFu && (uint64_t)last * 32ull < rankPixels) blocksWorthLaunching = false;
    }
    if (blocksWorthLaunching) {
        if (c->dBinHint) p.binHint = c->dBinHint + pass;
        if (!c->dLeftCmds) LR_HIP(hipMalloc((void**)&c->dLeftCmds, sizeof(ChordDrawCmd) * (size_t)c->cmdCapacity));
        p.leftCount = c->dCounts + 6 + pass; p.leftCmds = c->dLeftCmds;
        if (!c->inFrame || c->rasterCalls >= 2) LR_HIP(hipMemsetAsync(p.leftCount, 0, sizeof(uint32_t), c->stream));
    }
    p.orderKept = 0u;
    p.heavyHint = nullptr;
    static const bool directOn = [] { const char* e = getenv("CHORDVIS_TILE_DIRECT"); return !e || atoi(e) != 0; }();
    const bool laterOk = c->inFrame && !clearTiles && p.hzbFused && !c->depthOnly && c->dBinHint && !(c->debugFlags & ~(DBG_NO_BLOCKS | DBG_FORCE_BLOCKS | DBG_FORCE_HOT | 524288u));
    if (laterOk) p.heavyHint = c->dBinHint + 4 + pass;
    if (TILE_DIRECT && directOn && laterOk) {
        const uint32_t heavySeen = c->hBinHint[4 + pass], lightSeen = c->hBinHint[6 + pass];
        if (lightSeen != 0u && (heavySeen == 0u || (int32_t)(lightSeen - heavySeen) > 0)) {
            p.orderKept = 2u;
        }
    }
    static const int touchedEnv = [] { const char* e = getenv("CHORDVIS_TILE_TOUCHED"); return e ? atoi(e) : 1; }();
    p.tileTouched = nullptr;
    if (p.orderKept == 2u && touchedEnv != 0 && c->shard.ranks <= 1 && tiles <= 64u * 64u) {
        p.tileTouched = c->dFrameState->tileTouched + (size_t)pass * (CHORD_MAX_TILES / 32u);
        if (!c->inFrame || c->rasterCalls >= 2) LR_HIP(hipMemsetAsync(p.tileTouched, 0, sizeof(uint32_t) * ((tiles + 31u) / 32u), c->stream));
    }
    uint32_t blocks = (in.capacity + 3u) / 4u;
#ifndef SETUP_GRID_MULT
#define SETUP_GRID_MULT 1u
#endif
    const uint32_t maxBlocks = (uint32_t)c->numCUs * SETUP_MIN_WAVES * SETUP_GRID_MULT;
    if (blocks > maxBlocks) blocks = maxBlocks;
    if (blocks < 1) blocks = 1;
    const bool sh = c->shard.ranks > 1;
    stamp(c, S_HZBCULL);
    if (blocksWorthLaunching) {
        const uint32_t bb = std::max(1u, std::min((in.capacity + 3u) / 4u, (uint32_t)c->numCUs * BLOCKS_MIN_WAVES));
        const bool hot = (c->hBinHint && c->hBinHint[pass] >= SLOT_HOT) || (c->debugFlags & DBG_FORCE_HOT);
        if (hot) CHORD_LAUNCH(c, raster_setup_blocks_kernel<true>, dim3(bb), dim3(256), 0, c->stream, p);
        else     CHORD_LAUNCH(c, raster_setup_blocks_kernel<false>, dim3(bb), dim3(256), 0, c->stream, p);
    }
    static const int setupWide = [] { const char* e = getenv("CHORDVIS_SETUP_WIDE"); return e ? atoi(e) : 1; }();
    p.wideMax = setupWide > 1 ? (uint32_t)setupWide : TILE_DIRECT_MAX_CLUSTERS;
    c->setupWide[pass] = 0u;
    if (setupWide != 0 && p.orderKept == 2u && p.binInSetup && !blocksWorthLaunching && !sh) {
        const uint32_t wideBlocks = std::max(1u, std::min(std::max(in.capacity, 1u), (uint32_t)c->numCUs * SETUP_WIDE_WAVES));
        if (c->anyMasked) CHORD_LAUNCH(c, raster_setup_wide_kernel<true>, dim3(wideBlocks), dim3(256), 0, c->stream, p);
        else              CHORD_LAUNCH(c, raster_setup_wide_kernel<false>, dim3(wideBlocks), dim3(256), 0, c->stream, p);
        c->setupWide[pass] = 1u;
    } else if (c->anyMasked) CHORD_LAUNCH(c, raster_setup_kernel<true>, dim3(blocks), dim3(256), 0, c->stream, p);
    else                     CHORD_LAUNCH(c, raster_setup_kernel<false>, dim3(blocks), dim3(256), 0, c->stream, p);
    stamp(c, S_R_CLUSTER);
    if (!p.binInSetup) CHORD_LAUNCH(c, raster_clip_and_bin_large_kernel, dim3(CLIP_BLOCKS + (uint32_t)c->numCUs * 4u), dim3(256), 0, c->stream, p);
    bool makeOrder = p.orderKept != 2u;
    p.orderAll = 0u; p.tileOrderNext = nullptr;
    static const bool keepLaterOn = [] { const char* e = getenv("CHORDVIS_TILE_KEEP_LATER"); return !e || atoi(e) != 0; }();
    static const bool nextOn = [] { const char* e = getenv("CHORDVIS_TILE_NEXT"); return !e || atoi(e) != 0; }();
    const bool keepOk = TILE_ORDER_KEEP && c->orderKeepFrames && c->inFrame && !c->depthOnly && !(c->debugFlags & ~524288u);
    int slot = -1;
    if (keepOk && clearTiles && pass == 0u && c->dTileOrderKeep) slot = 0;
    else if (keepOk && keepLaterOn && laterOk && pass == 1u && c->dTileOrderKeep1) slot = 1;
    if (slot >= 0) {
        uint32_t& age = slot ? c->orderAge1 : c->orderAge;
        uint2* buf = reinterpret_cast<uint2*>(slot ? c->dTileOrderKeep1 : c->dTileOrderKeep);
        const size_t half = (size_t)1 + c->tileItemCap;
        p.orderAll = slot ? 1u : 0u;
        if (nextOn && p.orderKept == 2u) {
            age = 0xFFFFFFFFu; p.orderAll = 0u;
        } else if (nextOn) {
            uint32_t& flip = c->orderFlip[slot];
            p.tileOrder = buf + flip * half; p.tileOrderNext = buf + (flip ^ 1u) * half;
            if (age != 0xFFFFFFFFu) { p.orderKept = 1u; makeOrder = false; }
            age = 0u; flip ^= 1u;
        } else if (p.orderKept != 2u) {
            p.tileOrder = buf;
            if (age < c->orderKeepFrames) { age++; p.orderKept = 1u; makeOrder = false; }
            else age = 0u;
        } else p.orderAll = 0u;
    }
    if (makeOrder) CHORD_LAUNCH(c, raster_tile_order_kernel, dim3(1), dim3(1024), 0, c->stream, p);
    stamp(c, S_R_CLIP);
    const uint32_t slots = (uint32_t)c->numCUs * (CHORD_TILE_SHIFT == 6 ? 2u : 6u);
    const uint32_t tileBlocks = (p.tileOrderNext ? 1u : 0u) + ((clearTiles || (p.orderKept == 2u && !p.tileTouched) || p.orderAll) ? ((sh && clearTiles) ? min(tiles, max(c->shard.slotsPerRank, p.tileSlots + p.tileSlots / 2u)) : tiles)
                                                               : min(tiles, p.tileTouched && touchedEnv > 1 ? (uint32_t)touchedEnv : slots));
    if (c->anyMasked) {
        if (c->depthClamp && !sh) CHORD_LAUNCH(c, (raster_tile_kernel<false, true, true>), dim3(tileBlocks), dim3(TB), 0, c->stream, p);
        else if (sh)              CHORD_LAUNCH(c, (raster_tile_kernel<true, true, false>), dim3(tileBlocks), dim3(TB), 0, c->stream, p);
        else                      CHORD_LAUNCH(c, (raster_tile_kernel<false, true, false>), dim3(tileBlocks), dim3(TB), 0, c->stream, p);
    } else if (c->depthClamp && !sh) {
        CHORD_LAUNCH(c, (raster_tile_kernel<false, false, true>), dim3(tileBlocks), dim3(TB), 0, c->stream, p);
    } else {
        if (sh) CHORD_LAUNCH(c, (raster_tile_kernel<true, false, false>), dim3(tileBlocks), dim3(TB), 0, c->stream, p);
        else    CHORD_LAUNCH(c, (raster_tile_kernel<false, false, false>), dim3(tileBlocks), dim3(TB), 0, c->stream, p);
    }
    stamp(c, S_R_CHUNK);
    c->rasterCalls++;
    return hipSuccess;
#undef LR_HIP
}

}
```

Before: 3.470 Gtri/s.

## Split tile raster into fat and thin kernels by per-tile triangle count

The tile order now records where tiles with few bin entries begin. The frame's main opaque pass launches two kernels: the existing 512-thread tile kernel for heavy tiles, and a new 128-thread thin kernel with a smaller batch and unit list for light tiles, which walks the light tail of the order from the end. Block counts are sized from a mapped host hint written on the previous frame. The intent is to stop light tiles from occupying large workgroups and shared memory, which should raise occupancy. In exchange it adds a second launch, depends on a hint that can be a frame stale, and adds extra band loops in the HZB output for narrower workgroups.

```diff
diff --git a/chord_amd/csrc/chordvis_abi.cpp b/chord_amd/csrc/chordvis_abi.cpp
--- a/chord_amd/csrc/chordvis_abi.cpp
+++ b/chord_amd/csrc/chordvis_abi.cpp
@@ -171,6 +171,7 @@
     c->hBinHint[0] = 0u; c->hBinHint[1] = 0u;
     c->hBinHint[2] = 0xFFFFFFFFu; c->hBinHint[3] = 0xFFFFFFFFu;
     for (int k = 4; k < 8; k++) c->hBinHint[k] = 0u;
+    c->hBinHint[8] = 0xFFFFFFFFu;
     {
         const uint32_t vw = (c->width + 1) / 2, vh = (c->height + 1) / 2;
         if ((rc = dalloc(c, &c->dRangePartials, (size_t)((vw + 63) / 64) * ((vh + 3) / 4) * 2))) return rc;
diff --git a/chord_amd/csrc/kernels_raster.hip b/chord_amd/csrc/kernels_raster.hip
--- a/chord_amd/csrc/kernels_raster.hip
+++ b/chord_amd/csrc/kernels_raster.hip
@@ -70,6 +70,9 @@
     uint32_t* tileTouched;
     uint32_t debug;
     uint32_t wideMax;
+    uint32_t thinBucket;
+    uint32_t thinSplit;
+    uint32_t* thinHint;
 };
 #define ABL(p, flag) (RASTER_ABLATION && ((p).debug & (flag)) != 0u)
 #define DBG_NO_PIXELS   1u
@@ -1921,7 +1924,11 @@
     if (threadIdx.x == 0) {
         uint32_t acc = splitItems;
         for (int b = 0; b < 18; b++) { base[b] = acc; acc += hist[b]; }
-        order[0] = make_uint2((p.clearTiles || p.orderAll) ? acc : acc - hist[17], 0u);
+        base[18] = acc;
+        const uint32_t items = (p.clearTiles || p.orderAll) ? acc : acc - hist[17];
+        const uint32_t lightStart = min(base[min(p.thinBucket, 18u)], items);
+        order[0] = make_uint2(items, lightStart);
+        if (p.thinHint) *p.thinHint = items - lightStart;
         if (p.binHint) *p.binHint = longest;
         if (p.heavyHint) p.heavyHint[(splitItems != 0u || *p.count > TILE_DIRECT_MAX_CLUSTERS) ? 0 : 2] = p.binStamp;
         if (p.countHint) *p.countHint = *p.count;
@@ -1944,9 +1951,10 @@
     }
 }
 
+template <uint32_t NT>
 __device__ __noinline__ void tile_order_next_part(const RasterParams* q)
 {
-    tile_order_part<512u>(*q, q->tileOrderNext);
+    tile_order_part<NT>(*q, q->tileOrderNext);
 }
 
 __global__ __launch_bounds__(1024) void raster_tile_order_kernel(RasterParams p)
@@ -2093,6 +2101,7 @@
     }
 }
 
+template <uint32_t NTH = TB>
 __device__ __forceinline__ uint32_t block_scan_tb(uint32_t v, uint32_t* waveSums, uint32_t* total)
 {
     const uint32_t lane = threadIdx.x & 63u, wave = threadIdx.x >> 6;
@@ -2106,7 +2115,7 @@
     __syncthreads();
     uint32_t base = 0, tot = 0;
 #pragma unroll
-    for (uint32_t w = 0; w < TB / 64u; w++) { const uint32_t sw = waveSums[w]; if (w < wave) base += sw; tot += sw; }
+    for (uint32_t w = 0; w < NTH / 64u; w++) { const uint32_t sw = waveSums[w]; if (w < wave) base += sw; tot += sw; }
     *total = tot;
     return base + incl - v;
 }
@@ -2130,7 +2139,8 @@
 #ifndef TILE_UNIT_CAP
 #define TILE_UNIT_CAP UNIT_CAP
 #endif
-struct EntrySoA { uint32_t w[ENTRY_WORDS][TILE_BATCH]; };
+template <uint32_t BATCH> struct EntrySoAT { uint32_t w[ENTRY_WORDS][BATCH]; };
+using EntrySoA = EntrySoAT<TILE_BATCH>;
 #define EF_KIND_SHIFT 24
 
 template <typename E_t>
@@ -2203,7 +2213,8 @@
     return max(k1 - kFirst + 1, 0);
 }
 
-__device__ __forceinline__ uint32_t entry_store(EntrySoA& en, uint32_t t, const TriSetup& ts, bool narrow,
+template <class En>
+__device__ __forceinline__ uint32_t entry_store(En& en, uint32_t t, const TriSetup& ts, bool narrow,
                                                 int32_t ox, int32_t oy, int32_t x0, int32_t y0, int32_t x1, int32_t y1,
                                                 bool masked = false, uint32_t recIndex = 0u)
 {
@@ -2309,8 +2320,8 @@
     }
 }
 
-template <bool MASKED, bool DEPTH>
-__device__ __forceinline__ int32_t entry_unit(const RasterParams& p, const EntrySoA& en, unsigned long long* tile, uint32_t e, uint32_t row, uint32_t seg,
+template <bool MASKED, bool DEPTH, class En>
+__device__ __forceinline__ int32_t entry_unit(const RasterParams& p, const En& en, unsigned long long* tile, uint32_t e, uint32_t row, uint32_t seg,
                                            int32_t ox, int32_t oy, bool noPixels)
 {
     const uint32_t box = en.w[11][e];
@@ -2344,8 +2355,8 @@
     }
 }
 
-template <bool DEPTH>
-__device__ __forceinline__ void entry_unit_masked(const RasterParams& p, const EntrySoA& en, unsigned long long* tile, uint32_t e, uint32_t row, uint32_t seg,
+template <bool DEPTH, class En>
+__device__ __forceinline__ void entry_unit_masked(const RasterParams& p, const En& en, unsigned long long* tile, uint32_t e, uint32_t row, uint32_t seg,
                                                   int32_t ox, int32_t oy, bool noPixels)
 {
     const uint32_t box = en.w[11][e];
@@ -2384,16 +2395,16 @@
     return t;
 }
 
-template <bool INTERIOR, bool SH>
+template <bool INTERIOR, bool SH, uint32_t NTH = TB>
 __device__ __forceinline__ void tile_out_and_hzb_body(const TileOutParams& p, const unsigned long long* tile, float* sM2, uint32_t* sRange,
                                                       uint32_t tileId, uint32_t slotId, uint32_t binLength, int32_t ox, int32_t oy, int32_t tw, int32_t th)
 {
-    static_assert(TILE == 64 && TB == 512, "wave w <-> pixel rows 8w..8w+7");
+    static_assert(TILE == 64 && NTH >= 64u && 512u % NTH == 0u, "band b <-> pixel rows 8b..8b+7, eight bands over the workgroup's waves");
     const ChordHZBDesc& d = p.hzbDesc;
     const uint32_t tX = tileId % p.tilesX, tY = tileId / p.tilesX;
     uint32_t tid = threadIdx.x;
     asm volatile("" : "+v"(tid));
-    const uint32_t lane = tid & 63u, wave = tid >> 6, half = lane >> 5, l = lane & 31u;
+    const uint32_t lane = tid & 63u, wave0 = tid >> 6, half = lane >> 5, l = lane & 31u;
     uint16_t* exA = SH && p.hzbExA ? p.hzbExA + (size_t)slotId * CHORD_HZB_SLOT_HALVES : nullptr;
     uint16_t* exB = SH ? p.hzbExB + (size_t)slotId * CHORD_HZB_FINAL_SLOT_HALVES : nullptr;
     auto vw = [&](uint32_t lv) { return min(max(1u, d.width >> lv), (((d.srcWidth - 1u) >> 1) >> lv) + 1u); };
@@ -2419,6 +2430,9 @@
     };
     const uint32_t visBase = SH ? slotId << (2 * TILE_SHIFT) : (uint32_t)oy * (uint32_t)p.Wi + (uint32_t)ox;
     const uint32_t visPitch = SH ? (uint32_t)TILE : (uint32_t)p.Wi;
+#pragma unroll
+    for (uint32_t bandStep = 0; bandStep < 512u / NTH; bandStep++) {
+    const uint32_t wave = wave0 + bandStep * (NTH / 64u);
     uint32_t rmin = 0xFFFFFFFFu, rmax = 0u;
     float m1n = 0.0f, m1x = 0.0f;
 #pragma unroll
@@ -2469,8 +2483,9 @@
         rmax = max(rmax, (uint32_t)__shfl_down(rmax, off, 64));
     }
     if (lane == 0u) { sRange[wave * 2u] = rmin; sRange[wave * 2u + 1u] = rmax; }
+    }
     __syncthreads();
-    if (wave == 0u) {
+    if (wave0 == 0u) {
         const uint32_t x = lane & 7u, y = lane >> 3;
         float n3 = sM2[lane], x3 = sM2[64u + lane];
         n3 = fminf(n3, __shfl_xor(n3, 1, 64)); x3 = fmaxf(x3, __shfl_xor(x3, 1, 64));
@@ -2485,7 +2500,7 @@
             put(5u, 0u, 0u, n3, x3);
             uint32_t lo = 0xFFFFFFFFu, hi = 0u;
 #pragma unroll
-            for (uint32_t w = 0; w < TB / 64u; w++) { lo = min(lo, sRange[2u * w]); hi = max(hi, sRange[2u * w + 1u]); }
+            for (uint32_t w = 0; w < 8u; w++) { lo = min(lo, sRange[2u * w]); hi = max(hi, sRange[2u * w + 1u]); }
             if (SH) {
                 uint32_t* tail = reinterpret_cast<uint32_t*>(exB + CHORD_HZB_FINAL_RANGE_OFFSET);
                 const uint32_t before = p.clearTiles ? 0u : tail[2];
@@ -2497,7 +2512,7 @@
     }
 }
 
-template <bool SH>
+template <bool SH, uint32_t NTH = TB>
 __device__ __forceinline__ void tile_out_and_hzb(const unsigned long long* tile, float* sM2, uint32_t* sRange,
                                                  uint32_t tileId, uint32_t slotId, uint32_t binLength, int32_t ox, int32_t oy, int32_t tw, int32_t th)
 {
@@ -2506,8 +2521,8 @@
     const uint32_t tX = tileId % p.tilesX, tY = tileId / p.tilesX;
     const uint32_t vw0 = min(max(1u, d.width), ((d.srcWidth - 1u) >> 1) + 1u), vh0 = min(max(1u, d.height), ((d.srcHeight - 1u) >> 1) + 1u);
     const bool interior = tw == TILE && th == TILE && d.mipCount > 5u && (tX + 1u) * 32u <= vw0 && (tY + 1u) * 32u <= vh0;
-    if (interior) tile_out_and_hzb_body<true, SH>(p, tile, sM2, sRange, tileId, slotId, binLength, ox, oy, tw, th);
-    else tile_out_and_hzb_body<false, SH>(p, tile, sM2, sRange, tileId, slotId, binLength, ox, oy, tw, th);
+    if (interior) tile_out_and_hzb_body<true, SH, NTH>(p, tile, sM2, sRange, tileId, slotId, binLength, ox, oy, tw, th);
+    else tile_out_and_hzb_body<false, SH, NTH>(p, tile, sM2, sRange, tileId, slotId, binLength, ox, oy, tw, th);
 }
 
 __device__ __noinline__ bool merge_slices(unsigned long long* tile, unsigned long long* slab, uint32_t* ticket, uint32_t slices,
@@ -2623,14 +2638,16 @@
 #ifndef TILE_MIN_BLOCKS
 #define TILE_MIN_BLOCKS 4
 #endif
-template <bool SH, bool MASKED, bool DEPTH>
-__global__ __launch_bounds__(TB, TILE_MIN_BLOCKS) void raster_tile_kernel(RasterParams p)
-{
+template <bool SH, bool MASKED, bool DEPTH, uint32_t NTH, uint32_t BATCH, uint32_t UCAP, bool THIN>
+__device__ __forceinline__ void raster_tile_body(const RasterParams& p)
+{
+    static_assert(!THIN || (!SH && !MASKED && !DEPTH), "the thin form is the opaque single-GPU main view's");
+    static_assert(BATCH <= NTH && BATCH <= 512u && NTH <= 512u, "unit words hold the entry's thread in 9 bits");
     __shared__ __align__(16) unsigned long long tile[TILE * TPITCH];
-    __shared__ EntrySoA prm;
-    __shared__ uint32_t unitList[TILE_UNIT_CAP];
+    __shared__ EntrySoAT<BATCH> prm;
+    __shared__ uint32_t unitList[UCAP];
     __shared__ uint32_t offs[16];
-    __shared__ uint32_t waveSums[2][TB / 64];
+    __shared__ uint32_t waveSums[2][NTH / 64];
     __shared__ uint32_t chunkTab[64];
     __shared__ uint32_t sTicket;
     if (ABL(p, DBG_TILE_EXIT) && !p.clearTiles) return;
@@ -2639,13 +2656,16 @@
     const uint32_t tilesAll = p.tilesX * p.tilesY;
     const uint32_t wg0 = blockIdx.x - (p.tileOrderNext != nullptr ? 1u : 0u);
     if (p.tileOrderNext && blockIdx.x == 0u) {
-        tile_order_next_part(kernel_args());
+        if (THIN) tile_order_part<NTH>(p, p.tileOrderNext);
+        else tile_order_next_part<NTH>(kernel_args());
         return;
     }
     const bool direct = p.orderKept == 2u;
     uint2 firstItem = make_uint2(wg0, 0u);
     uint32_t active = tilesAll;
-    if (!direct) { firstItem = p.tileOrder[1u + min(wg0, tilesAll - 1u)]; active = p.tileOrder[0].x; }
+    uint32_t top = 0u;
+    if (THIN) { const uint2 hdr = p.tileOrder[0]; firstItem = p.tileOrder[1u + (tilesAll - 1u - min(wg0, tilesAll - 1u))]; top = hdr.x; active = hdr.x - min(hdr.y, hdr.x); }
+    else if (!direct) { firstItem = p.tileOrder[1u + min(wg0, tilesAll - 1u)]; const uint2 hdr = p.tileOrder[0]; active = p.thinSplit ? min(hdr.y, hdr.x) : hdr.x; }
     else if (p.tileTouched) {
         uint32_t touched, tail;
         firstItem.x = touched_tile(p.tileTouched, wg0, gridDim.x, touched, tail);
@@ -2656,11 +2676,12 @@
     const uint32_t oi = oiw & 0x7FFFFFFFu;
     uint32_t tix = threadIdx.x;
     asm volatile("" : "+v"(tix));
-    const uint2 itemCount = (oiw >> 31) == 0u ? firstItem : (direct ? make_uint2(oi + tilesAll - active, 0u) : p.tileOrder[1u + oi]);
+    const uint2 itemCount = THIN ? (((oiw >> 31) == 0u && top == tilesAll) ? firstItem : p.tileOrder[top - oi])
+                                 : (oiw >> 31) == 0u ? firstItem : (direct ? make_uint2(oi + tilesAll - active, 0u) : p.tileOrder[1u + oi]);
     const uint32_t item = itemCount.x;
-    const uint32_t tileId = item & 0xFFFu, slice = (item >> 12) & 0x3FFu, slices = (item >> 22) + 1u;
+    const uint32_t tileId = item & 0xFFFu, slice = THIN ? 0u : (item >> 12) & 0x3FFu, slices = THIN ? 1u : (item >> 22) + 1u;
     const uint32_t* bin = p.tileBins + (size_t)tileId * p.binCap;
-    const bool entryThread = TILE_BATCH == TB || tix < TILE_BATCH;
+    const bool entryThread = BATCH == NTH || tix < BATCH;
     uint32_t countWord = itemCount.y, wordSpec = 0xFFFFFFFFu;
     if (p.orderKept) {
         if (entryThread) wordSpec = bin[tix];
@@ -2705,9 +2726,9 @@
     const bool mergeSlices = slices > 1u && (p.clearTiles || rmw);
     if (!(rmw && !mergeSlices)) {
         static_assert((TILE * TPITCH) % 2 == 0, "whole 16-byte words");
-        for (uint32_t i = tix; i < TILE * TPITCH / 2; i += TB) reinterpret_cast<ulonglong2*>(tile)[i] = make_ulonglong2(0ull, 0ull);
+        for (uint32_t i = tix; i < TILE * TPITCH / 2; i += NTH) reinterpret_cast<ulonglong2*>(tile)[i] = make_ulonglong2(0ull, 0ull);
     } else
-    for (uint32_t i = tix, visBase = vis_base(); i < TILE * TILE / 2; i += TB) {
+    for (uint32_t i = tix, visBase = vis_base(); i < TILE * TILE / 2; i += NTH) {
         const int32_t ly = (int32_t)(i >> (TILE_SHIFT - 1)), lx = (int32_t)(i & (TILE / 2 - 1)) * 2;
         ulonglong2 v = make_ulonglong2(0ull, 0ull);
         if (ly < th && lx < tw) {
@@ -2733,7 +2754,7 @@
     if (early) {
         nameNext = record_name(word0);
         if (nameNext != 0xFFFFFFFFu) FETCH_REC(nameNext, nq0, nq1, nq2);
-        if (entryThread && k0 + TILE_BATCH < n) idxNext = record_name(bin[k0 + TILE_BATCH]);
+        if (entryThread && k0 + BATCH < n) idxNext = record_name(bin[k0 + BATCH]);
     }
     __syncthreads();
     PHASE(0);
@@ -2742,7 +2763,7 @@
     const uint32_t chunksAll = n > p.binCap ? (n - p.binCap + CHORD_BIN_CHUNK - 1u) >> CHORD_BIN_CHUNK_SHIFT : 0u;
     auto window_load = [&](uint32_t from, uint32_t to) {
         const RasterParams* q = kernel_args();
-        for (uint32_t j = from + tix; j < to; j += TB) {
+        for (uint32_t j = from + tix; j < to; j += NTH) {
             const unsigned long long e = scalar_load(&q->binChunkTab)[(size_t)tileId * scalar_load(&q->binMaxChunks) + j];
             chunkTab[j & 63u] = (uint32_t)(e >> 32) == scalar_load(&q->binStamp) ? (uint32_t)e : CHORD_BIN_CHUNK_INVALID;
         }
@@ -2776,10 +2797,10 @@
         const unsigned long long* blockPool = scalar_load(&kernel_args()->blockPool);
         const uint32_t blockLimit = blockCap * CHORD_LIST_SHARDS;
         uint32_t giNext = lo + tix < n ? binWord(lo + tix) : 0xFFFFFFFFu;
-        for (uint32_t base = lo; base < n; base += TB) {
+        for (uint32_t base = lo; base < n; base += NTH) {
             window_advance(base);
             const uint32_t gi = giNext;
-            giNext = base + TB + tix < n ? binWord(base + TB + tix) : 0xFFFFFFFFu;
+            giNext = base + NTH + tix < n ? binWord(base + NTH + tix) : 0xFFFFFFFFu;
             const bool isBlock = gi != 0xFFFFFFFFu && gi >= CHORD_REC_BLOCK && (gi & CHORD_REC_INDEX_MASK) < blockLimit;
             uint2 hdr = make_uint2(0u, 0u);
             if (isBlock) hdr = *reinterpret_cast<const uint2*>(blockPool + (size_t)(gi & CHORD_REC_INDEX_MASK) * 2u);
@@ -2797,7 +2818,7 @@
         idxNext = entryThread && k0 < n ? binEntry(k0) : 0xFFFFFFFFu;
         nameNext = idxNext;
         if (nameNext != 0xFFFFFFFFu) FETCH_REC(nameNext, nq0, nq1, nq2);
-        idxNext = entryThread && k0 + TILE_BATCH < n ? binEntry(k0 + TILE_BATCH) : 0xFFFFFFFFu;
+        idxNext = entryThread && k0 + BATCH < n ? binEntry(k0 + BATCH) : 0xFFFFFFFFu;
     }
     auto batch_setup = [&](const uint4 q0, const uint4 q1, const uint4 q2, const uint32_t name) -> uint32_t {
         const bool have = name != 0xFFFFFFFFu && !ABL(p, DBG_NO_ENTRY);
@@ -2844,7 +2865,7 @@
         uint32_t total;
         const bool mine3 = MASKED && rows && ((prm.w[11][tix] >> EF_KIND_SHIFT) & 3u) == 3u;
         const uint32_t rowsN = mine3 ? 0u : rows, rowsM = mine3 ? rows : 0u;
-        const uint32_t offAll = block_scan_tb(rowsN | (rowsM << 16), waveSums[batchNo & 1u], &total);
+        const uint32_t offAll = block_scan_tb<NTH>(rowsN | (rowsM << 16), waveSums[batchNo & 1u], &total);
         const uint32_t offN = offAll & 0xFFFFu, offM = offAll >> 16, totalM = MASKED ? total >> 16 : 0u;
         total &= 0xFFFFu;
         PHASE(3);
@@ -2852,7 +2873,7 @@
             if (!n) return;
             const uint32_t box = prm.w[11][tix];
             const uint32_t nseg = ((((box >> 12) & 63u) - (box & 63u)) >> SEG_SHIFT) + 1u, y0l = (box >> 6) & 63u;
-            const uint32_t lo2 = max(off, r0), hi2 = min(off + n, r0 + TILE_UNIT_CAP);
+            const uint32_t lo2 = max(off, r0), hi2 = min(off + n, r0 + UCAP);
             if (lo2 < hi2) {
                 uint32_t j = lo2 - off;
                 uint32_t row = y0l + (nseg == 1u ? j : nseg == 2u ? j >> 1 : nseg == 4u ? j >> 2 : j / 3u);
@@ -2863,23 +2884,23 @@
                 }
             }
         };
-        for (uint32_t r0 = 0; r0 < total; r0 += TILE_UNIT_CAP) {
+        for (uint32_t r0 = 0; r0 < total; r0 += UCAP) {
             list_units(offN, rowsN, r0);
             __syncthreads();
-            const uint32_t nr = min(total - r0, (uint32_t)TILE_UNIT_CAP);
-            for (uint32_t ui = tix; ui < nr; ui += TB) {
+            const uint32_t nr = min(total - r0, (uint32_t)UCAP);
+            for (uint32_t ui = tix; ui < nr; ui += NTH) {
                 const uint32_t d = unitList[ui];
                 if (ABL(p, DBG_NO_UNITS)) continue;
                 const int32_t trips = entry_unit<MASKED, DEPTH>(p, prm, tile, d & 511u, (d >> 9) & 63u, (d >> 15) & 3u, ox, oy, noPixels);
                 if (prof) { cUnits++; cUnitIters += (uint32_t)trips; }
             }
-            if (r0 + TILE_UNIT_CAP < total || totalM) __syncthreads();
-        }
-        for (uint32_t r0 = 0; r0 < totalM; r0 += TILE_UNIT_CAP) {
+            if (r0 + UCAP < total || totalM) __syncthreads();
+        }
+        for (uint32_t r0 = 0; r0 < totalM; r0 += UCAP) {
             if (rowsM) {
                 const uint32_t box = prm.w[11][tix];
                 const uint32_t nseg = ((((box >> 12) & 63u) - (box & 63u)) >> MASKED_SEG_SHIFT) + 1u, y0l = (box >> 6) & 63u;
-                const uint32_t lo2 = max(offM, r0), hi2 = min(offM + rowsM, r0 + TILE_UNIT_CAP);
+                const uint32_t lo2 = max(offM, r0), hi2 = min(offM + rowsM, r0 + UCAP);
                 if (lo2 < hi2) {
                     const uint32_t j = lo2 - offM, g = j / nseg;
                     uint32_t row = y0l + g * MASKED_ROWS, seg = j - g * nseg;
@@ -2890,26 +2911,26 @@
                 }
             }
             __syncthreads();
-            const uint32_t nr = min(totalM - r0, (uint32_t)TILE_UNIT_CAP);
-            for (uint32_t ui = tix; ui < nr; ui += TB) {
+            const uint32_t nr = min(totalM - r0, (uint32_t)UCAP);
+            for (uint32_t ui = tix; ui < nr; ui += NTH) {
                 const uint32_t d = unitList[ui];
                 entry_unit_masked<DEPTH>(p, prm, tile, d & 511u, (d >> 9) & 63u, (d >> 15) & 7u, ox, oy, noPixels);
             }
-            if (r0 + TILE_UNIT_CAP < totalM) __syncthreads();
+            if (r0 + UCAP < totalM) __syncthreads();
         }
         total |= totalM;
         if (total) __syncthreads();
         PHASE(4);
     };
     uint32_t batchNo = 0;
-    for (uint32_t base = lo; base < n; base += TILE_BATCH, batchNo++) {
+    for (uint32_t base = lo; base < n; base += BATCH, batchNo++) {
         window_advance(base);
         const uint32_t k = base + tix;
         const uint4 q0 = nq0, q1 = nq1, q2 = nq2;
         const uint32_t name = nameNext;
         nameNext = idxNext;
         if (nameNext != 0xFFFFFFFFu) FETCH_REC(nameNext, nq0, nq1, nq2);
-        idxNext = entryThread && k + 2u * TILE_BATCH < n ? binEntry(k + 2u * TILE_BATCH) : 0xFFFFFFFFu;
+        idxNext = entryThread && k + 2u * BATCH < n ? binEntry(k + 2u * BATCH) : 0xFFFFFFFFu;
         batch_units(batch_setup(q0, q1, q2, name), batchNo);
     }
     __syncthreads();
@@ -2919,7 +2940,7 @@
         if (!merge_slices(tile, scalar_load(&q->tileSlabs) + (size_t)tileId * (TILE * TILE), &scalar_load(&q->tileCount)[(size_t)tileId * TC_STRIDE + TC_TICKET],
                           slices, &sTicket, &scalar_load(&q->counters)->overflow)) continue;
         if (rmw) {
-            for (uint32_t i = tix, visBase = vis_base(); i < TILE * TILE / 2; i += TB) {
+            for (uint32_t i = tix, visBase = vis_base(); i < TILE * TILE / 2; i += NTH) {
                 const int32_t ly = (int32_t)(i >> (TILE_SHIFT - 1)), lx = (int32_t)(i & (TILE / 2 - 1)) * 2;
                 if (ly >= th || lx >= tw) continue;
                 const unsigned long long* src = p.vis + (size_t)(visBase + (uint32_t)ly * visPitch + (uint32_t)lx);
@@ -2932,9 +2953,9 @@
 
     if (ABL(p, DBG_NO_OUT)) {
     } else if (p.hzbFused && !ABL(p, DBG_NO_HZB)) {
-        tile_out_and_hzb<SH>(tile, reinterpret_cast<float*>(&prm.w[0][0]), offs, tileId, slot_of_tile(), nAll, ox, oy, tw, th);
+        tile_out_and_hzb<SH, NTH>(tile, reinterpret_cast<float*>(&prm.w[0][0]), offs, tileId, slot_of_tile(), nAll, ox, oy, tw, th);
     } else if (p.clearTiles || p.hzbFused) {
-        for (uint32_t i = tix, visBase = vis_base(); i < TILE * TILE / 2; i += TB) {
+        for (uint32_t i = tix, visBase = vis_base(); i < TILE * TILE / 2; i += NTH) {
             const int32_t ly = (int32_t)(i >> (TILE_SHIFT - 1)), lx = (int32_t)(i & (TILE / 2 - 1)) * 2;
             if (ly >= th || lx >= tw) continue;
             const ulonglong2 v = make_ulonglong2(tile[ly * TPITCH + lx], tile[ly * TPITCH + lx + 1]);
@@ -2943,7 +2964,7 @@
             else dst[0] = v.x;
         }
     } else {
-        for (uint32_t i = tix, visBase = vis_base(); i < TILE * TILE; i += TB) {
+        for (uint32_t i = tix, visBase = vis_base(); i < TILE * TILE; i += NTH) {
             const int32_t ly = (int32_t)(i >> TILE_SHIFT), lx = (int32_t)(i & (TILE - 1));
             const unsigned long long v = tile[ly * TPITCH + lx];
             if (v != 0ull && ly < th && lx < tw) atomicMax(p.vis + (size_t)(visBase + (uint32_t)ly * visPitch + (uint32_t)lx), v);
@@ -2966,6 +2987,23 @@
 }
 #undef wgs
 #undef TILE_SKEW
+
+template <bool SH, bool MASKED, bool DEPTH>
+__global__ __launch_bounds__(TB, TILE_MIN_BLOCKS) void raster_tile_kernel(RasterParams p)
+{
+    raster_tile_body<SH, MASKED, DEPTH, TB, TILE_BATCH, TILE_UNIT_CAP, false>(p);
+}
+
+#ifndef TILE_THIN_TB
+#define TILE_THIN_TB 128
+#endif
+#define TILE_THIN_BATCH 64
+#define TILE_THIN_UNIT_CAP 512
+__global__ __launch_bounds__(TILE_THIN_TB, TILE_THIN_TB / 64) void raster_tile_thin_kernel(RasterParams p)
+{
+    raster_tile_body<false, false, false, TILE_THIN_TB, TILE_THIN_BATCH, TILE_THIN_UNIT_CAP, true>(p);
+}
+
 
 
 hipError_t launch_raster(ChordCtx* c, const CmdList& in, bool clearTiles)
@@ -3114,6 +3152,21 @@
     if (!p.binInSetup) CHORD_LAUNCH(c, raster_clip_and_bin_large_kernel, dim3(CLIP_BLOCKS + (uint32_t)c->numCUs * 4u), dim3(256), 0, c->stream, p);
     bool makeOrder = p.orderKept != 2u;
     p.orderAll = 0u; p.tileOrderNext = nullptr;
+#ifndef TILE_THIN_MAX
+#define TILE_THIN_MAX 64u
+#endif
+    static const int thinEnv = [] { const char* e = getenv("CHORDVIS_TILE_THIN"); return e ? atoi(e) : 1; }();
+    static const int thinMaxEnv = [] { const char* e = getenv("CHORDVIS_TILE_THIN_MAX"); return e ? atoi(e) : 0; }();
+    static const bool thinFirst = [] { const char* e = getenv("CHORDVIS_TILE_THIN_FIRST"); return e && atoi(e) != 0; }();
+    const bool thinOk = thinEnv != 0 && clearTiles && pass == 0u && c->inFrame && c->shard.ranks <= 1 && !c->anyMasked && !c->depthOnly && !c->depthClamp &&
+                        !c->debugFlags && !blocksWorthLaunching && p.orderKept != 2u && c->dBinHint;
+    p.thinBucket = 18u; p.thinSplit = 0u; p.thinHint = nullptr;
+    if (thinOk) {
+        const uint32_t thinMax = thinMaxEnv > 0 ? (uint32_t)thinMaxEnv : thinEnv > 1 ? (uint32_t)thinEnv : TILE_THIN_MAX;
+        uint32_t t = 0u;
+        while (t < 17u && (1u << t) < thinMax) t++;
+        p.thinBucket = 17u - t; p.thinHint = c->dBinHint + 8;
+    }
     static const bool keepLaterOn = [] { const char* e = getenv("CHORDVIS_TILE_KEEP_LATER"); return !e || atoi(e) != 0; }();
     static const bool nextOn = [] { const char* e = getenv("CHORDVIS_TILE_NEXT"); return !e || atoi(e) != 0; }();
     const bool keepOk = TILE_ORDER_KEEP && c->orderKeepFrames && c->inFrame && !c->depthOnly && !(c->debugFlags & ~524288u);
@@ -3143,7 +3196,18 @@
     const uint32_t slots = (uint32_t)c->numCUs * (CHORD_TILE_SHIFT == 6 ? 2u : 6u);
     const uint32_t tileBlocks = (p.tileOrderNext ? 1u : 0u) + ((clearTiles || (p.orderKept == 2u && !p.tileTouched) || p.orderAll) ? ((sh && clearTiles) ? min(tiles, max(c->shard.slotsPerRank, p.tileSlots + p.tileSlots / 2u)) : tiles)
                                                                : min(tiles, p.tileTouched && touchedEnv > 1 ? (uint32_t)touchedEnv : slots));
-    if (c->anyMasked) {
+    if (thinOk) {
+        RasterParams pf = p, pt = p;
+        pf.thinSplit = 1u; pt.thinSplit = 1u;
+        (thinFirst ? pt : pf).tileOrderNext = nullptr;
+        const uint32_t seen = c->hBinHint[8];
+        const uint32_t light = seen == 0xFFFFFFFFu ? tiles : min(seen, tiles);
+        const uint32_t fatBlocks = (pf.tileOrderNext ? 1u : 0u) + max(1u, seen == 0xFFFFFFFFu ? tiles : tiles - light);
+        const uint32_t thinBlocks = (pt.tileOrderNext ? 1u : 0u) + max(1u, light);
+        if (thinFirst) CHORD_LAUNCH(c, raster_tile_thin_kernel, dim3(thinBlocks), dim3(TILE_THIN_TB), 0, c->stream, pt);
+        CHORD_LAUNCH(c, (raster_tile_kernel<false, false, false>), dim3(fatBlocks), dim3(TB), 0, c->stream, pf);
+        if (!thinFirst) CHORD_LAUNCH(c, raster_tile_thin_kernel, dim3(thinBlocks), dim3(TILE_THIN_TB), 0, c->stream, pt);
+    } else if (c->anyMasked) {
         if (c->depthClamp && !sh) CHORD_LAUNCH(c, (raster_tile_kernel<false, true, true>), dim3(tileBlocks), dim3(TB), 0, c->stream, p);
         else if (sh)              CHORD_LAUNCH(c, (raster_tile_kernel<true, true, false>), dim3(tileBlocks), dim3(TB), 0, c->stream, p);
         else                      CHORD_LAUNCH(c, (raster_tile_kernel<false, true, false>), dim3(tileBlocks), dim3(TB), 0, c->stream, p);
```

Result: slower. 2.869 Gtri/s (-17.3%).
